# FKGSOFTWARE/TERRA-GAN

Measured on AMD Instinct MI355X. Metric: DSM tiles/sec train-step (G+D) at 256x256 bs=16, higher is better.
Workload: dtype f32; 1 GPU; BASELINE configs[1]: 256x256 1-ch DSM tiles, batch 16 per GPU, fp32, PConv-UNet G + PatchGAN D + L1/VGG-perceptual/TV/boundary(0.5) losses + 2x Adam; global_batch=16, tile=256, parallelism=single-gpu, launch=eager, vgg_weights=deterministic stand-in (ImageNet weights not fetchable offline; same FLOPs), vgg_trunk=forward Winograd F(2x2,3x3), dgrads F(4x4,3x3) (DESIGN 2b)

## Files before the change

### include/terragan_hip.h

```cpp
#ifndef TERRAGAN_HIP_H
#define TERRAGAN_HIP_H

#include <stddef.h>
#include <stdint.h>

#ifdef __cplusplus
extern "C" {
#endif

typedef void* tg_stream_t;

enum { TG_OK = 0, TG_ERR_ARG = -1, TG_ERR_LAUNCH = -2, TG_ERR_WS = -3 };
enum { TG_ACT_NONE = 0, TG_ACT_RELU = 1, TG_ACT_LEAKY = 2 };
enum { TG_PREC_F32 = 0, TG_PREC_BF16 = 1, TG_PREC_F32_WINO4 = 2 };

typedef struct TgConv {
    int32_t B, H, W, Cin;
    int32_t Ho, Wo, Cout;
    int32_t k, stride, pad;
    int32_t precision;
} TgConv;

int tg_version(void);
const char* tg_last_error(void);


size_t tg_conv_fwd_ws_bytes(const TgConv* g);
int tg_conv_fwd(const TgConv* g, const float* x, const float* in_mask, const float* w,
                const float* bias, const float* ratio, int act, float slope, float* y,
                float* ws, size_t ws_bytes, tg_stream_t stream);

size_t tg_conv_dgrad_ws_bytes(const TgConv* g);
int tg_conv_dgrad(const TgConv* g, const float* dy, const float* w, const float* in_mask,
                  float* dx, int accumulate, float* ws, size_t ws_bytes, tg_stream_t stream);
int tg_conv_dgrad_gated(const TgConv* g, const float* dy, const float* w, const float* in_mask,
                        const float* x_act, int act, float slope, float* dx, float* ws,
                        size_t ws_bytes, tg_stream_t stream);

enum { TG_WPREP_FWD = 0, TG_WPREP_DGRAD = 1 };
size_t tg_conv_wprep_bytes(const TgConv* g, int mode);
int tg_conv_wprep(const TgConv* g, int mode, const float* w, float* wprep, tg_stream_t stream);
size_t tg_conv_wprep_item_bytes(void);
int tg_conv_wprep_item(const TgConv* g, int mode, const float* w, float* wprep, void* item_out);
int tg_conv_wprep_run(const void* items_dev, int n, tg_stream_t stream);
int tg_conv_fwd_p(const TgConv* g, const float* x, const float* in_mask, const float* w, const float* wprep,
                  const float* bias, const float* ratio, int act, float slope, float* y, float* ws,
                  size_t ws_bytes, tg_stream_t stream);
int tg_conv_fwd_pool(const TgConv* g, const float* x, const float* in_mask, const float* w, const float* wprep,
                     const float* bias, const float* ratio, int act, float slope, float* y, float* pool_y, float* ws,
                     size_t ws_bytes, tg_stream_t stream);
int tg_conv_pool_code_supported(const TgConv* g);
int tg_conv_fwd_pool_code(const TgConv* g, const float* x, const float* w, const float* wprep, const float* bias,
                          float* pool_y, unsigned char* code, float* ws, size_t ws_bytes, tg_stream_t stream);
int tg_maxpool2_bwd_code(const float* dout, const unsigned char* code, int B, int Ho, int Wo, int C, float* dx,
                         tg_stream_t stream);
typedef struct TgSparseMap {
    const uint32_t* bits;
    const int32_t* list;
    const int32_t* count;
    const uint64_t* pix;
    int32_t nb, tiles_y, tiles_x, _pad;
} TgSparseMap;
size_t tg_vgg_sparse_map_bytes(int nb, int H, int W, const char* plan);
int tg_vgg_sparse_map(const float* x, const float* mask, int nb, int H, int W, const char* plan, void* buf, size_t buf_bytes,
                      int* ticket, TgSparseMap* maps, tg_stream_t stream);
int tg_conv_dgrad_sparse(const TgConv* g, const float* dy, const float* w, const float* wprep, const float* x_act, int act,
                         float slope, const uint32_t* gate_bits, float* dx, const TgSparseMap* sp, float* ws, size_t ws_bytes,
                         tg_stream_t stream);
int tg_conv_dgrad_sparse_planned(const TgConv* g, int gate, const TgSparseMap* sp);
int tg_maxpool2_bwd_code_sparse(const float* dout, const unsigned char* code, int B, int Ho, int Wo, int C, float* dx,
                                const TgSparseMap* sp, tg_stream_t stream);
int tg_conv_fwd_sparse(const TgConv* g, const float* x, const float* w, const float* wprep, const float* bias, int act,
                       float slope, float* y, float* pool_y, unsigned char* code, const TgSparseMap* sp, float* ws,
                       size_t ws_bytes, tg_stream_t stream);
typedef struct TgBnAct {
    const float *mean, *rstd, *gamma, *beta;
    int32_t act;
    float slope;
} TgBnAct;
int tg_conv_bnin_supported(const TgConv* g, int wgrad);
int tg_conv_fwd_bnin(const TgConv* g, const float* x, const TgBnAct* bn, const float* w, const float* bias, int act,
                     float slope, float* y, float* ws, size_t ws_bytes, tg_stream_t stream);
int tg_conv_wgrad_bnin(const TgConv* g, const float* x, const TgBnAct* bn, const float* dy, float* dw, float* db, float* ws,
                       size_t ws_bytes, tg_stream_t stream);
int tg_conv_dgrad_p(const TgConv* g, const float* dy, const float* w, const float* wprep, const float* in_mask,
                    const float* x_act, int act, float slope, float* dx, int accumulate, float* ws,
                    size_t ws_bytes, tg_stream_t stream);
int tg_relu_gate_pack(const float* a, int64_t rows, int C, uint32_t* bits, tg_stream_t stream);
int tg_conv_dgrad_gbits(const TgConv* g, const float* dy, const float* w, const float* wprep, const float* in_mask,
                        const uint32_t* gate_bits, float* dx, int accumulate, float* ws, size_t ws_bytes, tg_stream_t stream);

int tg_set_cu_reserve(int cus);
int tg_set_work_stealing(int mode);

size_t tg_conv_wgrad_ws_bytes(const TgConv* g);
int tg_conv_wgrad(const TgConv* g, const float* x, const float* in_mask, const float* dy,
                  float* dw, float* db, float* ws, size_t ws_bytes, tg_stream_t stream);

int tg_fold_cin(const float* w3, int cout, int taps, int cin, float* w1, tg_stream_t stream);


int tg_mask_update(const float* mask, int B, int H, int W, int k, int stride, int pad, int Ho,
                   int Wo, float* mask_out, float* ratio, tg_stream_t stream);
int tg_mask_up_merge(const float* up_mask, const float* skip_mask, int B, int h, int w, int H,
                     int W, float* out, tg_stream_t stream);

#define TG_MASK_PYRAMID_MAX 24
typedef struct TgMaskOp {
    int kind, H, W, Ho, Wo, k, stride, pad;
    const float* in;
    const float* in2;
    float* out;
    float* out2;
} TgMaskOp;
typedef struct TgMaskPyramid {
    int nops, _pad;
    TgMaskOp op[TG_MASK_PYRAMID_MAX];
} TgMaskPyramid;
int tg_mask_pyramid(const TgMaskPyramid* pm, int B, tg_stream_t stream);


size_t tg_bn_ws_bytes(int64_t rows, int C);
int tg_bn_stats(const float* y, int64_t rows, int C, float eps, float momentum, float* save_mean,
                float* save_rstd, float* running_mean, float* running_var,
                int64_t* num_batches_tracked, float* ws, size_t ws_bytes, tg_stream_t stream);
int tg_bn_fwd(const float* y, int64_t rows, int C, float eps, float momentum, const float* gamma,
              const float* beta, int act, float slope, float* save_mean, float* save_rstd,
              float* running_mean, float* running_var, int64_t* num_batches_tracked, float* out,
              float* ws, size_t ws_bytes, tg_stream_t stream);
int tg_bn_eval_stats(const float* running_mean, const float* running_var, int C, float eps,
                     float* mean, float* rstd, tg_stream_t stream);
int tg_bn_act_fwd(const float* y, int64_t rows, int C, const float* mean, const float* rstd,
                  const float* gamma, const float* beta, int act, float slope, float* out,
                  tg_stream_t stream);
int tg_bn_act_bwd(const float* dout, const float* y, int64_t rows, int C, const float* mean,
                  const float* rstd, const float* gamma, const float* beta, int act, float slope,
                  const float* ratio, float* dy, float* dgamma, float* dbeta, float* dbias, float* ws,
                  size_t ws_bytes, tg_stream_t stream);
int tg_bn_bwd_conv1_supported(int64_t rows, int C);
size_t tg_bn_conv1_ws_bytes(int64_t rows, int C);
int tg_bn_act_bwd_conv1(const float* dz, const float* w, int B, int H, int W, const float* y, int C, const float* mean,
                        const float* rstd, const float* gamma, const float* beta, int act, float slope, const float* ratio,
                        float* dy, float* dgamma, float* dbeta, float* dbias, float* ws, size_t ws_bytes, tg_stream_t stream);
int tg_act_bwd(const float* dout, const float* out, int64_t rows, int C, int act, float slope,
               const float* ratio, float* din, tg_stream_t stream);


int tg_upcat_fwd(const float* up, const float* skip, const float* out_mask, int B, int h, int w,
                 int Cu, int H, int W, int Cs, float* out, tg_stream_t stream);
int tg_upcat_bn_supported(int B, int h, int w, int Cu, int H, int W, int Cs);
int tg_upcat_fwd_bn(const float* up, const TgBnAct* bn, const float* skip, const float* out_mask, int B, int h, int w,
                    int Cu, int H, int W, int Cs, float* out, tg_stream_t stream);
int tg_upcat_bwd(const float* dout, int B, int h, int w, int Cu, int H, int W, int Cs, float* dup,
                 float* dskip, tg_stream_t stream);


int tg_sigmoid_composite_fwd(const float* logits, const float* x, const float* mask, int64_t n,
                             float* out, tg_stream_t stream);
int tg_sigmoid_composite_bwd(const float* dout, const float* logits, const float* mask, int64_t n,
                             float* dlogits, float* dx, tg_stream_t stream);

int tg_maxpool2_fwd(const float* x, int B, int H, int W, int C, float* out, tg_stream_t stream);
int tg_maxpool2_bwd(const float* dout, const float* x, int B, int H, int W, int C, int relu_gate,
                    float* dx, tg_stream_t stream);


size_t tg_pixel_loss_ws_bytes(int B, int H, int W);
int tg_pixel_losses(const float* pred, const float* target, const float* mask,
                    const float* l1_weight, int B, int H, int W,
                    float w_l1, float w_tv, float w_bnd, float bnd_eps, const float* gscale,
                    float* out5, float* dpred, int accumulate, float* ws, size_t ws_bytes,
                    tg_stream_t stream);

size_t tg_reduce_ws_bytes(int64_t n);
int tg_l1_mean(const float* a, const float* b, int64_t n, float coef, const float* gscale,
               float* out1, float* da, float* ws, size_t ws_bytes, tg_stream_t stream);
int tg_l1_mean_relu(const float* a, const float* b, int64_t n, float coef, const float* gscale, float* out1, float* da,
                    float* ws, size_t ws_bytes, tg_stream_t stream);

int tg_bce_logits(const float* z, int64_t n, float target, float coef, const float* gscale,
                  float* out1, float* dz, float* ws, size_t ws_bytes, tg_stream_t stream);


int tg_adam(float* p, const float* g, float* m, float* v, int64_t n, double lr, double beta1,
            double beta2, double eps, int step, float grad_scale, tg_stream_t stream);

typedef struct TgAdamSeg {
    float* p;
    const float* g;
    float* m;
    float* v;
    int64_t n;
} TgAdamSeg;
int tg_adam_multi(const TgAdamSeg* segs_dev, const int32_t* work_dev, int nwork, int chunk_elems,
                  double lr, double beta1, double beta2, double eps, int step, float grad_scale,
                  tg_stream_t stream);

int tg_adam_scalars(double lr, double beta1, double beta2, int step, float* out2_host);
int tg_write_floats(float* dst_dev, int n, const float* vals_host, tg_stream_t stream);
int tg_adam_multi_s(const TgAdamSeg* segs_dev, const int32_t* work_dev, int nwork, int chunk_elems,
                    double beta1, double beta2, double eps, const float* scal_dev, float grad_scale,
                    tg_stream_t stream);

int tg_axpby(const float* x, float a, float b, float* y, int64_t n, tg_stream_t stream);
int tg_lincomb(const float* x, float a, const float* y, float b, float* out, int64_t n,
               tg_stream_t stream);
int tg_mul(const float* a, const float* b, float* out, int64_t n, tg_stream_t stream);
int tg_mul_keep(const float* a, const float* b, float* out, float* a_copy, int64_t n, tg_stream_t stream);
size_t tg_bn_grouped_ws_bytes(int64_t rows_per_group, int groups, int C);
int tg_bn_fwd_grouped(const float* y, int64_t rows_per_group, int groups, int C, float eps, const float* gamma,
                      const float* beta, int act, float slope, float* save_mean, float* save_rstd, float* out,
                      float* ws, size_t ws_bytes, tg_stream_t stream);
int tg_bn_act_bwd_grouped(const float* dout, const float* y, int64_t rows_per_group, int groups, int C,
                          const float* mean, const float* rstd, const float* gamma, const float* beta, int act,
                          float slope, float* dy, float* dgamma, float* dbeta, float* dbias, float* ws,
                          size_t ws_bytes, tg_stream_t stream);
int tg_bn_running_update_multi(const float* save_mean, const float* save_rstd, int64_t rows_per_group, int C,
                               float eps, float momentum, const int* order, int norder, float* running_mean,
                               float* running_var, int64_t* num_batches_tracked, tg_stream_t stream);
int tg_bn_running_update(const float* save_mean, const float* save_rstd, int64_t rows, int C,
                         float eps, float momentum, float* running_mean, float* running_var,
                         int64_t* num_batches_tracked, tg_stream_t stream);
int tg_nchw_to_nhwc(const float* x, int B, int C, int H, int W, float* y, tg_stream_t stream);
int tg_nhwc_to_nchw(const float* x, int B, int C, int H, int W, float* y, tg_stream_t stream);


size_t tg_quality_metrics_ws_bytes(int64_t imgs, int H, int W);
int tg_quality_metrics(const float* pred, const float* target, const float* mask, int64_t imgs, int H, int W,
                       float* out9, float* ws, size_t ws_bytes, tg_stream_t stream);

int tg_u8_to_tiles(const uint8_t* img_u8, const uint8_t* mask_u8, int64_t n, float* img_f32, float* mask_f32,
                   tg_stream_t stream);

typedef struct TgRasterPlan {
    int32_t H, W;
    int32_t wh, ww;
    int32_t overlap;
    int32_t ny, nx;
} TgRasterPlan;

int tg_raster_window_stats(const float* dem, const float* mask, const TgRasterPlan* plan, int use_nodata, float nodata,
                           float* lo, float* hi, int32_t* counts, tg_stream_t stream);
int tg_raster_gather(const float* dem, const float* mask, const TgRasterPlan* plan, int use_nodata, float nodata,
                     const float* lo, const float* hi, const int32_t* win_idx, int n, float* x, float* m, tg_stream_t stream);
int tg_raster_blend(const float* dem, const float* mask, const TgRasterPlan* plan, int use_nodata, float nodata,
                    const float* lo, const float* hi, const int32_t* run_of_window, const float* wout, int n_run, float* out,
                    int32_t* unfilled, tg_stream_t stream);

enum { TG_HOLE_RECT = 0, TG_HOLE_ELLIPSE = 1, TG_HOLE_STROKE = 2 };
int tg_hole_masks(const int32_t* prims, const int32_t* offsets, int n, int side, float* mask, tg_stream_t stream);
// ... 71 lines not shown
```

### terra-gan_amd/csrc/igemm.hip

```cpp
#include <atomic>
#include <stdlib.h>
#include <string.h>

#include <mutex>
#include <vector>

#include "common.h"

struct ProfRec {
    hipEvent_t a, b;
    int kind;
    double flops, bytes;
    int M, N, K, C, splits, cfg;
    char tag[32];
};
static std::mutex g_prof_mu;
static bool g_prof_on = false;
static std::vector<ProfRec> g_prof;
static thread_local char g_prof_tag[32] = "";

struct ProfScope {
    bool on = false;
    ProfRec r{};
    hipStream_t s;
    ProfScope(hipStream_t st, int kind, double flops, double bytes, int M = 0, int N = 0, int K = 0, int C = 0, int splits = 1,
              int cfg = 0)
        : s(st) {
        if (!g_prof_on) return;
        on = true;
        r.kind = kind; r.flops = flops; r.bytes = bytes;
        r.M = M; r.N = N; r.K = K; r.C = C; r.splits = splits; r.cfg = cfg;
        memcpy(r.tag, g_prof_tag, sizeof(r.tag));
        (void)hipEventCreate(&r.a);
        (void)hipEventCreate(&r.b);
        (void)hipEventRecord(r.a, s);
    }
    ~ProfScope() {
        if (!on) return;
        (void)hipEventRecord(r.b, s);
        std::lock_guard<std::mutex> lk(g_prof_mu);
        g_prof.push_back(r);
    }
};

static thread_local double g_alg_scale = 1.0;
struct AlgScale {
    double prev;
    explicit AlgScale(double sc) : prev(g_alg_scale) { g_alg_scale = sc; }
    ~AlgScale() { g_alg_scale = prev; }
};

extern "C" int tg_prof_enable(int on) {
    std::lock_guard<std::mutex> lk(g_prof_mu);
    g_prof_on = on != 0;
    return TG_OK;
}
extern "C" int tg_prof_tag(const char* tag) {
    strncpy(g_prof_tag, tag ? tag : "", sizeof(g_prof_tag) - 1);
    g_prof_tag[sizeof(g_prof_tag) - 1] = 0;
    return TG_OK;
}
extern "C" int tg_prof_dump(const char* path) {
    std::lock_guard<std::mutex> lk(g_prof_mu);
    FILE* f = fopen(path, "w");
    if (!f) { tg_set_error("tg_prof_dump: cannot open %s", path); return TG_ERR_ARG; }
    fprintf(f, "kind,cfg,M,N,K,C,splits,ms,gflop,alg_mb,tag\n");
    for (auto& r : g_prof) {
        (void)hipEventSynchronize(r.b);
        float t = 0.f;
        (void)hipEventElapsedTime(&t, r.a, r.b);
        fprintf(f, "%d,%d,%d,%d,%d,%d,%d,%.5f,%.4f,%.3f,%s\n", r.kind, r.cfg, r.M, r.N, r.K, r.C, r.splits, t, r.flops / 1e9,
                r.bytes / 1e6, r.tag);
    }
    fclose(f);
    return TG_OK;
}
extern "C" int tg_prof_summary(int kind, double* total_ms, int64_t* launches, double* flops, double* bytes) {
    std::lock_guard<std::mutex> lk(g_prof_mu);
    double ms = 0, fl = 0, by = 0;
    int64_t n = 0;
    std::vector<ProfRec> keep;
    for (auto& r : g_prof) {
        if (r.kind != kind) { keep.push_back(r); continue; }
        (void)hipEventSynchronize(r.b);
        float t = 0.f;
        (void)hipEventElapsedTime(&t, r.a, r.b);
        ms += t; fl += r.flops; by += r.bytes; ++n;
        (void)hipEventDestroy(r.a);
        (void)hipEventDestroy(r.b);
    }
    g_prof.swap(keep);
    if (total_ms) *total_ms = ms;
    if (launches) *launches = n;
    if (flops) *flops = fl;
    if (bytes) *bytes = by;
    return TG_OK;
}

#include "igemm_params.h"

struct LdsOptIn {
    std::mutex mu;
    bool done[64] = {};
};
static int lds_opt_in(LdsOptIn& st, const void* kern, size_t lds, const char* who) {
    int dev = 0;
    (void)hipGetDevice(&dev);
    std::lock_guard<std::mutex> lk(st.mu);
    if (dev >= 0 && dev < 64 && st.done[dev]) return TG_OK;
    hipError_t e = hipFuncSetAttribute(kern, hipFuncAttributeMaxDynamicSharedMemorySize, (int)lds);
    if (e != hipSuccess) {
        tg_set_error("%s: hipFuncSetAttribute(%zu) failed: %s", who, lds, hipGetErrorString(e));
        return TG_ERR_LAUNCH;
    }
    if (dev >= 0 && dev < 64) st.done[dev] = true;
    return TG_OK;
}

constexpr int WINO_PLAN_CUS = 256;
static std::atomic<int> g_cu_reserve{0};
static int wino_cus() {
    const int c = 256 - g_cu_reserve.load(std::memory_order_relaxed);
    return c < 8 ? 8 : c;
}
extern "C" int tg_set_cu_reserve(int cus) {
    TG_REQUIRE(cus >= 0 && cus <= 128, "tg_set_cu_reserve: %d out of range [0,128]", cus);
    g_cu_reserve.store(cus, std::memory_order_relaxed);
    return TG_OK;
}

static std::atomic<int> g_work_stealing{0};
extern "C" int tg_set_work_stealing(int mode) {
    TG_REQUIRE(mode >= 0 && mode <= 2, "tg_set_work_stealing: mode %d not in {0, 1, 2}", mode);
    g_work_stealing.store(mode, std::memory_order_relaxed);
    return TG_OK;
}
constexpr int WQ_HOST_Z = 16, WQ_HOST_INTS = 8 * WQ_HOST_Z + 8, WQ_POOL_BLOCKS = 64;
static int* wino_queue_block(hipStream_t s, int splits, int total_work) {
    static const int env_mode = getenv("TG_WORK_STEALING") ? atoi(getenv("TG_WORK_STEALING")) : 0;
    const int set_mode = g_work_stealing.load(std::memory_order_relaxed);
    const int mode = set_mode ? set_mode : env_mode;
    if (mode <= 0 || splits > WQ_HOST_Z) return nullptr;
    if (mode == 1 && total_work < 2 * wino_cus()) return nullptr;
    static std::mutex mu;
    static std::vector<std::pair<std::pair<int, hipStream_t>, int*>> blocks;
    static int* pools[64] = {};
    static int used[64] = {};
    int dev = 0;
    if (hipGetDevice(&dev) != hipSuccess || dev < 0 || dev >= 64) return nullptr;
    std::lock_guard<std::mutex> lk(mu);
    for (auto& b : blocks)
        if (b.first.first == dev && b.first.second == s) return b.second;
    hipStreamCaptureStatus st = hipStreamCaptureStatusNone;
    if (hipStreamIsCapturing(s, &st) != hipSuccess || st != hipStreamCaptureStatusNone) {
        if (!pools[dev]) return nullptr;
    }
    if (!pools[dev]) {
        if (hipMalloc(reinterpret_cast<void**>(&pools[dev]), (size_t)WQ_POOL_BLOCKS * WQ_HOST_INTS * sizeof(int)) != hipSuccess) { pools[dev] = nullptr; return nullptr; }
        if (hipMemset(pools[dev], 0, (size_t)WQ_POOL_BLOCKS * WQ_HOST_INTS * sizeof(int)) != hipSuccess) return nullptr;
    }
    if (used[dev] >= WQ_POOL_BLOCKS) return nullptr;
    int* blk = pools[dev] + (size_t)used[dev]++ * WQ_HOST_INTS;
    blocks.push_back({{dev, s}, blk});
    return blk;
}

static int choose_splits(long tiles, int max_splits, int slots) {
    if (max_splits < 1) max_splits = 1;
    if (tiles >= 4L * slots) return 1;
    int best = 1;
    double best_eff = 0.0;
    for (int sp = 1; sp <= max_splits; ++sp) {
        const long blocks = tiles * sp;
        const long rounds = (blocks + slots - 1) / slots;
        const double eff = (double)blocks / ((double)rounds * slots);
        if (eff > best_eff + 1e-9) { best_eff = eff; best = sp; }
        if (blocks >= slots && eff >= 0.92) return sp;
        if (blocks >= 6L * slots) break;
    }
    return best;
}


static int choose_splits_k(long tiles, int max_splits, int slots, long ksteps, double slab_steps = 0.0) {
    if (max_splits < 1) max_splits = 1;
    int best = 1;
    double best_cost = 1e300;
    for (int sp = 1; sp <= max_splits; ++sp) {
        const long blocks = tiles * sp;
        const long rounds = (blocks + slots - 1) / slots;
        const double cost = (double)rounds * ((double)((ksteps + sp - 1) / sp) + 4.0) + slab_steps * (double)blocks;
        if (cost < best_cost * 0.995) { best_cost = cost; best = sp; }
    }
    return best;
}

__device__ __forceinline__ int cdiv_dev(int a, int b) { return (a + b - 1) / b; }
__device__ __forceinline__ int xcd_remap(int id, int total) {
    const int xcd = id & 7, slot = id >> 3;
    const int qd = total >> 3, rm = total & 7;
    return (xcd < rm ? xcd * (qd + 1) : rm * (qd + 1) + (xcd - rm) * qd) + slot;
}

__device__ __forceinline__ f32x4 epilogue4(const IGemmParams& p, f32x4 o, size_t pix, int nb, const f32x4* gv_pre = nullptr,
                                           const float* rs_pre = nullptr, const f32x4* bias_pre = nullptr) {
    const float rs = rs_pre ? *rs_pre : (p.rowscale ? p.rowscale[pix] : 1.f);
    if (bias_pre) o += *bias_pre;
    else if (p.bias) o += *reinterpret_cast<const f32x4*>(p.bias + nb);
    o *= rs;
#pragma unroll
    for (int e = 0; e < 4; ++e) o[e] = apply_act(o[e], p.act, p.slope);
    if (p.gate) {
        const f32x4 gv = gv_pre ? *gv_pre : *reinterpret_cast<const f32x4*>(p.gate + pix * p.N + nb);
#pragma unroll
        for (int e = 0; e < 4; ++e) o[e] *= gv[e] > 0.f ? 1.f : (p.gate_act == TG_ACT_LEAKY ? p.gate_slope : 0.f);
    }
    if (p.accumulate) o += *reinterpret_cast<const f32x4*>(p.dst + pix * p.N + nb);
    return o;
}

__device__ __forceinline__ size_t dst_pixel(const IGemmParams& p, int m) {
    if (p.ds == 1 && p.OH == p.DH && p.OW == p.DW) return (size_t)m;
    int ox = m % p.OW;
    int t = m / p.OW;
    int oy = t % p.OH;
    int b = t / p.OH;
    return ((size_t)b * p.DH + (oy * p.ds + p.dy0)) * p.DW + (ox * p.ds + p.dx0);
}

template <int WAVES_M, int WAVES_N, int WM, int WN, bool SCALAR, bool BF16>
__device__ __forceinline__ void igemm_body(const IGemmParams& p, const int bz) {
    constexpr int BM = WAVES_M * WM * 32, BN = WAVES_N * WN * 32, LDK = 36;
    constexpr int A_LOADS = BM / 32, B_LOADS = BN / 32;
    static_assert(WAVES_M * WAVES_N == 4, "4 waves per workgroup");
    extern __shared__ __attribute__((aligned(16))) float smem[];
    float* As = smem;
    float* Bs = smem + 2 * BM * LDK;
    constexpr int LDH = 40;
    __bf16* Ah = reinterpret_cast<__bf16*>(smem);
    __bf16* Bh = Ah + 2 * BM * LDH;

    const int tid = threadIdx.x, lane = tid & 63, wave = tid >> 6;
    const int wm = wave / WAVES_N, wn = wave % WAVES_N;
    const int m0 = blockIdx.x * BM, n0 = blockIdx.y * BN;
    if (m0 >= p.M) return;
    const int kc = tid & 7, r0 = tid >> 3;

    int rb[A_LOADS], ry[A_LOADS], rx[A_LOADS];
    bool rv[A_LOADS];
#pragma unroll
    for (int i = 0; i < A_LOADS; ++i) {
        int m = m0 + r0 + 32 * i;
        rv[i] = m < p.M;
        int mm = rv[i] ? m : 0;
        int ox = mm % p.OW;
        int t = mm / p.OW;
        int oy = t % p.OH;
        rb[i] = t / p.OH;
        ry[i] = oy * p.ss + p.sy0;
        rx[i] = ox * p.ss + p.sx0;
    }

    const int t_begin = bz * p.steps_per_split;
    const int t_end = min(p.T, t_begin + p.steps_per_split);

    f32x4 ra[A_LOADS], rw[B_LOADS];
    float rmk[A_LOADS];

    int l_ty = 0, l_tx = 0, l_ch = 0;
    if constexpr (!SCALAR) {
        const int tap0 = t_begin / p.nchunks;
        l_ch = t_begin - tap0 * p.nchunks;
        l_ty = tap0 / p.TW;
        l_tx = tap0 - l_ty * p.TW;
    }
    int g_c0 = 0, g_dyy = 0, g_dxx = 0, g_widx = 0;
    bool g_cv = false;
    auto gbegin = [&]() {
        g_c0 = l_ch * 32 + 4 * kc;
        g_dyy = l_ty * p.tstep;
        g_dxx = l_tx * p.tstep;
        g_widx = ((p.ky0 + l_ty * p.kstep) * p.KW + (p.kx0 + l_tx * p.kstep)) * p.C + g_c0;
        g_cv = g_c0 < p.C;
        if (++l_ch == p.nchunks) {
            l_ch = 0;
            if (++l_tx == p.TW) { l_tx = 0; ++l_ty; }
        }
// ... 924 lines not shown
static size_t align_up(size_t v, size_t a) { return (v + a - 1) / a * a; }
#include "wino22.inc"
static size_t conv_wino_floats(const TgConv* g) {
    if (wino22_fwd_geom_ok(g) || wino22_dgrad_geom_ok(g)) return wino22_u_floats(g);
    if (g->k != 3 || g->stride != 1 || (g->Cin % 8) != 0 || (g->Cout % 8) != 0) return 0;
    if (g->precision == TG_PREC_F32_WINO4) return align_up(wino44_u_floats(g->Cout, g->Cin), 64);
    return align_up(wino_u_floats(g->Cout, g->Cin), 64);
}

__global__ __launch_bounds__(256) void s2d_kernel(const float* __restrict__ x, const float* __restrict__ mask, float* __restrict__ x2,
                                                  int B, int H, int W, int C) {
    const int C4 = C >> 2;
    const int64_t total = (int64_t)B * H * W * C4;
    for (int64_t idx = (int64_t)blockIdx.x * 256 + threadIdx.x; idx < total; idx += (int64_t)gridDim.x * 256) {
        const int c4 = (int)(idx % C4);
        int64_t pix = idx / C4;
        const int xw = (int)(pix % W);
        int64_t t = pix / W;
        const int yh = (int)(t % H);
        const int b = (int)(t / H);
        f32x4 v = *reinterpret_cast<const f32x4*>(x + pix * C + 4 * c4);
        if (mask) v *= mask[pix];
        const int64_t p2 = ((int64_t)b * (H >> 1) + (yh >> 1)) * (W >> 1) + (xw >> 1);
        *reinterpret_cast<f32x4*>(x2 + p2 * (4 * C) + ((yh & 1) * 2 + (xw & 1)) * C + 4 * c4) = v;
    }
}
__global__ __launch_bounds__(256) void d2s_kernel(const float* __restrict__ dx2, const float* __restrict__ mask, float* __restrict__ dx,
                                                  int B, int H, int W, int C, int accumulate) {
    const int C4 = C >> 2;
    const int64_t total = (int64_t)B * H * W * C4;
    for (int64_t idx = (int64_t)blockIdx.x * 256 + threadIdx.x; idx < total; idx += (int64_t)gridDim.x * 256) {
        const int c4 = (int)(idx % C4);
        int64_t pix = idx / C4;
        const int xw = (int)(pix % W);
        int64_t t = pix / W;
        const int yh = (int)(t % H);
        const int b = (int)(t / H);
        const int64_t p2 = ((int64_t)b * (H >> 1) + (yh >> 1)) * (W >> 1) + (xw >> 1);
        f32x4 v = *reinterpret_cast<const f32x4*>(dx2 + p2 * (4 * C) + ((yh & 1) * 2 + (xw & 1)) * C + 4 * c4);
        if (mask) v *= mask[pix];
        float* o = dx + pix * C + 4 * c4;
        if (accumulate) v += *reinterpret_cast<const f32x4*>(o);
        *reinterpret_cast<f32x4*>(o) = v;
    }
}
__global__ __launch_bounds__(256) void w5x5_s2d_kernel(const float* __restrict__ src, float* __restrict__ dst, int Cout, int C, int to3) {
    const int64_t total = to3 ? (int64_t)Cout * 36 * C : (int64_t)Cout * 25 * C;
    for (int64_t idx = (int64_t)blockIdx.x * 256 + threadIdx.x; idx < total; idx += (int64_t)gridDim.x * 256) {
        const int c = (int)(idx % C);
        int64_t t = idx / C;
        if (to3) {
            const int ph = (int)(t % 4), tap = (int)((t / 4) % 9), co = (int)(t / 36);
            const int ky = 2 * (tap / 3) + (ph >> 1), kx = 2 * (tap % 3) + (ph & 1);
            dst[idx] = (ky < 5 && kx < 5) ? src[((int64_t)co * 25 + ky * 5 + kx) * C + c] : 0.f;
        } else {
            const int k = (int)(t % 25), co = (int)(t / 25);
            const int ky = k / 5, kx = k % 5;
            dst[idx] = src[(((int64_t)co * 9 + (ky >> 1) * 3 + (kx >> 1)) * 4 + (ky & 1) * 2 + (kx & 1)) * C + c];
        }
    }
}
static bool s2d_ok(const TgConv* g) {
    static const bool off = getenv("TG_NO_WINO") != nullptr || getenv("TG_NO_S2D") != nullptr;
    if (off || (g->precision == TG_PREC_BF16 && getenv("TG_NO_WINO16"))) return false;
    return g->k == 5 && g->stride == 2 && g->pad == 2 && (g->H % 2) == 0 && (g->W % 2) == 0 && (g->Cin % 16) == 0 &&
           (g->Cout % 64) == 0 && g->Ho >= 32 && g->Wo >= 32 && g->Ho == g->H / 2 && g->Wo == g->W / 2;
}
static TgConv s2d_geom(const TgConv* g) {
    TgConv g2 = *g;
    g2.H = g->H / 2; g2.W = g->W / 2; g2.Cin = 4 * g->Cin; g2.k = 3; g2.stride = 1; g2.pad = 1;
    return g2;
}
static size_t s2d_x_floats(const TgConv* g) { return align_up((size_t)g->B * g->H * g->W * g->Cin, 64); }
static size_t s2d_w_floats(const TgConv* g) { return align_up((size_t)g->Cout * 36 * g->Cin, 64); }

static size_t splitk_room_floats(size_t out) {
    const size_t cap = (size_t)64 << 20;
    return out * 64 < cap ? out * 64 : cap;
}
static size_t min_floats(size_t a, size_t b) { return a < b ? a : b; }

extern "C" size_t tg_conv_fwd_ws_bytes(const TgConv* g) {
    if (!g) return 0;
    const size_t out = (size_t)g->B * g->Ho * g->Wo * g->Cout;
    size_t base = (splitk_room_floats(out) + conv_wino_floats(g)) * sizeof(float);
    if (s2d_ok(g)) {
        const TgConv g2 = s2d_geom(g);
        base = (s2d_x_floats(g) + s2d_w_floats(g)) * sizeof(float) + tg_conv_fwd_ws_bytes(&g2);
    }
    return base;
}

static IGemmParams conv_fwd_params(const TgConv* g) {
    IGemmParams p = {};
    p.B = g->B; p.IH = g->H; p.IW = g->W; p.C = g->Cin;
    p.OH = g->Ho; p.OW = g->Wo; p.N = g->Cout; p.M = g->B * g->Ho * g->Wo;
    p.DH = g->Ho; p.DW = g->Wo; p.ds = 1; p.dy0 = 0; p.dx0 = 0;
    p.TH = g->k; p.TW = g->k; p.ss = g->stride; p.tstep = 1; p.sy0 = -g->pad; p.sx0 = -g->pad;
    p.KW = g->k; p.kstep = 1; p.ky0 = 0; p.kx0 = 0;
    p.Kfull = g->k * g->k * g->Cin;
    p.bf16 = g->precision == TG_PREC_BF16;
    p.wino4 = g->precision == TG_PREC_F32_WINO4;
    p.Ktot = p.TH * p.TW * p.C; p.nchunks = cdiv(p.C, 32);
    p.T = (p.C % 4) ? cdiv(p.Ktot, 32) : p.TH * p.TW * p.nchunks;
    return p;
}
static IGemmParams conv_dgrad_s1_params(const TgConv* g) {
    IGemmParams p = {};
    p.B = g->B; p.IH = g->Ho; p.IW = g->Wo; p.C = g->Cout;
    p.OH = g->H; p.OW = g->W; p.N = g->Cin; p.M = g->B * g->H * g->W;
    p.DH = g->H; p.DW = g->W; p.ds = 1;
    p.ky0 = 0; p.kx0 = 0; p.TH = g->k; p.TW = g->k; p.ss = g->stride; p.tstep = -1; p.sy0 = g->pad; p.sx0 = g->pad;
    p.KW = g->k; p.kstep = 1; p.Kfull = g->k * g->k * g->Cout;
    p.bf16 = g->precision == TG_PREC_BF16;
    p.wino4 = g->precision == TG_PREC_F32_WINO4;
    return p;
}
static bool wino_fwd_geom_ok(const TgConv* g) { return wino_geom_ok(conv_fwd_params(g)); }
static bool wino_dgrad_geom_ok(const TgConv* g) { return wino_geom_ok(conv_dgrad_s1_params(g)); }

static int launch_wino_s1(IGemmParams& p, float* ws, size_t head, size_t avail, size_t room, hipStream_t s, const char* who) {
    if (wino44_ok(p)) {
        TG_REQUIRE(!p.pool_only, "%s: wino44_kernel cannot write the pool in place of the output", who);
        return launch_wino44(p, s);
    }
    if (wino44_prepared_unusable(p)) {
        TG_REQUIRE(ws && aligned16(ws) && avail >= head, "%s: workspace too small to re-prepare the weights (%zu < %zu floats)", who,
                   avail, head);
        p.wino_u = ws;
        p.wino_ready = 0;
        p.ws = ws + head;
        avail -= head;
    }
    return launch_wino(p, min_floats(avail, room), s);
}

static size_t dgrad_wt_floats(const TgConv* g);
extern "C" size_t tg_conv_wprep_bytes(const TgConv* g, int mode) {
    if (!g) return 0;
    if (s2d_ok(g)) {
        const TgConv g2 = s2d_geom(g);
        return s2d_w_floats(g) * sizeof(float) + tg_conv_wprep_bytes(&g2, mode);
    }
    if (mode == TG_WPREP_FWD) return wino_fwd_geom_ok(g) || wino22_fwd_geom_ok(g) ? conv_wino_floats(g) * sizeof(float) : 0;
    if (mode == TG_WPREP_DGRAD) return dgrad_wt_floats(g) * sizeof(float);
    return 0;
}

struct FwdExtras {
    float* pool_dst = nullptr;
    unsigned char* pool_code = nullptr;
    const BnIn* in_bn = nullptr;
    const TgSparseMap* sparse = nullptr;
    int pool_fused = 0;
};
static int conv_fwd_impl(const TgConv* g, const float* x, const float* in_mask, const float* w, float* wprep, int prep,
                         const float* bias, const float* ratio, int act, float slope, float* y, float* ws, size_t ws_bytes,
                         tg_stream_t stream, float* pool_y = nullptr, FwdExtras* ex = nullptr) {
    if (pool_y) {
        TG_REQUIRE(g && x && y && prep >= 0 && (g->Ho % 2) == 0 && (g->Wo % 2) == 0 && aligned16(pool_y),
                   "tg_conv_fwd_pool: even output sizes and a 16-byte aligned pool_y expected");
        int fused = 0;
        if (!s2d_ok(g) && !wino22_fwd_geom_ok(g)) {
            FwdExtras e;
            e.pool_dst = pool_y;
            e.sparse = ex ? ex->sparse : nullptr;
            const int rc1 = conv_fwd_impl(g, x, in_mask, w, wprep, prep, bias, ratio, act, slope, y, ws, ws_bytes, stream, nullptr, &e);
            if (rc1) return rc1;
            fused = e.pool_fused;
        } else if (int rc1 = conv_fwd_impl(g, x, in_mask, w, wprep, prep, bias, ratio, act, slope, y, ws, ws_bytes, stream)) {
            return rc1;
        }
        return fused ? TG_OK : tg_maxpool2_fwd(y, g->B, g->Ho, g->Wo, g->Cout, pool_y, stream);
    }
    int rc = check_conv(g, "tg_conv_fwd");
    if (rc) return rc;
    TG_REQUIRE(w && (prep < 0 || (x && y)), "tg_conv_fwd: null pointer");
    TG_REQUIRE(aligned16(x) && aligned16(w) && aligned16(y) && aligned16(wprep), "tg_conv_fwd: pointers must be 16-byte aligned");
    TG_REQUIRE(prep == 0 || wprep != nullptr, "tg_conv_fwd: prepared weights expected");
    const bool ws_ok = ws && aligned16(ws) && ws_bytes >= tg_conv_fwd_ws_bytes(g);
    if (s2d_ok(g) && (prep < 0 || ws_ok)) {
        hipStream_t s = (hipStream_t)stream;
        const TgConv g2 = s2d_geom(g);
        float* x2 = ws;
        float* w2 = prep ? wprep : ws + s2d_x_floats(g);
        float* ws2 = ws ? ws + s2d_x_floats(g) + s2d_w_floats(g) : nullptr;
        if (prep < 0 && g_wprep_capture) {
            const int rc2 = conv_fwd_impl(&g2, nullptr, nullptr, w2, wprep + s2d_w_floats(g), -1, nullptr, nullptr, 0, 0.f, nullptr, nullptr,
                                          0, stream);
            if (rc2 == TG_OK && g_wprep_captured == 1 && g_wprep_capture->kind == 1) {
                g_wprep_capture->kind = 4; g_wprep_capture->w = w; g_wprep_capture->taps = g->Cin;
            } else {
                g_wprep_captured = -1;
            }
            return rc2;
        }
        if (prep <= 0) {
            hipLaunchKernelGGL(w5x5_s2d_kernel, dim3(ew_grid((int64_t)g->Cout * 36 * g->Cin, 256)), dim3(256), 0, s, w, w2, g->Cout, g->Cin, 1);
            TG_CHECK_LAUNCH("w5x5_s2d_kernel");
        }
        if (prep >= 0) {
            hipLaunchKernelGGL(s2d_kernel, dim3(ew_grid((int64_t)g->B * g->H * g->W * (g->Cin / 4), 256)), dim3(256), 0, s, x, in_mask, x2,
                               g->B, g->H, g->W, g->Cin);
            TG_CHECK_LAUNCH("s2d_kernel");
        }
        AlgScale sc(25.0 / 36.0);
        return conv_fwd_impl(&g2, x2, nullptr, w2, prep ? wprep + s2d_w_floats(g) : nullptr, prep, bias, ratio, act, slope, y, ws2,
                             ws ? ws_bytes - (s2d_x_floats(g) + s2d_w_floats(g)) * sizeof(float) : 0, stream);
    }
    TG_REQUIRE(!(s2d_ok(g) && prep > 0), "tg_conv_fwd: workspace too small for the prepared 5x5 stride-2 path");
    IGemmParams p = conv_fwd_params(g);
    p.src = x; p.amask = in_mask; p.wmat = w; p.bias = bias; p.rowscale = ratio; p.dst = y; p.ws = ws;
    p.act = act; p.slope = slope; p.accumulate = 0;
    size_t ws_floats = ws ? ws_bytes / sizeof(float) : 0;
    const size_t uf = conv_wino_floats(g);
    const size_t room = splitk_room_floats((size_t)p.M * p.N);
    if (wino22_fwd_geom_ok(g) && (prep || (ws_floats >= uf && aligned16(ws)))) {
        p.w_raw = w;
        p.wino_u = prep ? wprep : ws;
        p.wino_ready = prep;
        if (!prep) {
            p.ws = ws + uf;
            ws_floats -= uf;
        }
        return launch_wino22(g, p, 0, min_floats(ws_floats, room), (hipStream_t)stream);
    }
    const bool wino = wino_fwd_geom_ok(g) && (prep || (ws_floats >= uf && aligned16(ws)));
    if (prep < 0 && !wino) return TG_OK;
    if (ex) {
        p.pool_dst = ex->pool_dst;
        p.pool_code = ex->pool_code;
        p.pool_only = ex->pool_code != nullptr;
        p.sparse = ex->sparse;
        if (ex->in_bn) {
            p.in_bn = *ex->in_bn;
            TG_REQUIRE(smallconv_bnin_fwd_ok(p), "tg_conv_fwd_bnin: geometry not supported (ask tg_conv_bnin_supported first)");
        }
    }
    if (wino) {
        p.w_raw = w; p.w_sn = (long)p.Kfull; p.w_sk = 1; p.w_stap = g->Cin;
        p.wino_u = prep ? wprep : ws;
        p.wino_ready = prep;
        if (!prep) {
            p.ws = ws + uf;
            ws_floats -= uf;
        }
        rc = launch_wino_s1(p, ws, uf, ws_floats, room, (hipStream_t)stream, "tg_conv_fwd");
    } else {
        ws_floats = min_floats(ws_floats, room);
        plan_splits(p, ws_floats);
        rc = launch_igemm(p, (hipStream_t)stream, ws_floats);
    }
    if (ex) ex->pool_fused = p.pool_done;
    return rc;
}
extern "C" int tg_conv_fwd_pool(const TgConv* g, const float* x, const float* in_mask, const float* w, const float* wprep,
                                const float* bias, const float* ratio, int act, float slope, float* y, float* pool_y, float* ws,
                                size_t ws_bytes, tg_stream_t stream) {
    TG_REQUIRE(pool_y, "tg_conv_fwd_pool: null pointer");
    return conv_fwd_impl(g, x, in_mask, w, const_cast<float*>(wprep), wprep ? 1 : 0, bias, ratio, act, slope, y, ws, ws_bytes, stream,
                         pool_y);
}
extern "C" int tg_conv_pool_code_supported(const TgConv* g) {
    if (!g || (g->precision != TG_PREC_F32 && g->precision != TG_PREC_BF16) || !wino_fwd_geom_ok(g) || s2d_ok(g) || (g->Ho & 1) ||
        (g->Wo & 1) || getenv("TG_NO_POOL_CODE"))
        return 0;
    IGemmParams p = conv_fwd_params(g);
    float pooled;
    p.pool_dst = &pooled;
    return wino_plan(p, splitk_room_floats((size_t)p.M * p.N)).pool ? 1 : 0;
}
static int conv_fwd_pool_code(const TgConv* g, const float* x, const float* w, const float* wprep, const float* bias, float* pool_y,
                              unsigned char* code, const TgSparseMap* sp, float* ws, size_t ws_bytes, tg_stream_t stream) {
    TG_REQUIRE(pool_y && code && aligned16(pool_y) && (reinterpret_cast<uintptr_t>(code) & 3) == 0, "tg_conv_fwd_pool_code: bad pointers");
    TG_REQUIRE(tg_conv_pool_code_supported(g), "tg_conv_fwd_pool_code: geometry not supported (ask tg_conv_pool_code_supported first)");
    FwdExtras e;
    e.pool_dst = pool_y;
    e.pool_code = code;
    e.sparse = sp;
    const int rc = conv_fwd_impl(g, x, nullptr, w, const_cast<float*>(wprep), wprep ? 1 : 0, bias, nullptr, TG_ACT_RELU, 0.f, pool_y, ws,
                                 ws_bytes, stream, nullptr, &e);
    if (rc) return rc;
    TG_REQUIRE(e.pool_fused, "tg_conv_fwd_pool_code: internal: the launch did not take the fused path");
    return TG_OK;
}
extern "C" int tg_conv_fwd_pool_code(const TgConv* g, const float* x, const float* w, const float* wprep, const float* bias,
                                     float* pool_y, unsigned char* code, float* ws, size_t ws_bytes, tg_stream_t stream) {
    return conv_fwd_pool_code(g, x, w, wprep, bias, pool_y, code, nullptr, ws, ws_bytes, stream);
}
extern "C" int tg_conv_fwd_sparse(const TgConv* g, const float* x, const float* w, const float* wprep, const float* bias, int act,
                                  float slope, float* y, float* pool_y, unsigned char* code, const TgSparseMap* sp, float* ws,
                                  size_t ws_bytes, tg_stream_t stream) {
    if (code) {
        TG_REQUIRE(act == TG_ACT_RELU, "tg_conv_fwd_sparse: the pool code needs a ReLU output");
        return conv_fwd_pool_code(g, x, w, wprep, bias, pool_y, code, sp, ws, ws_bytes, stream);
    }
    FwdExtras e;
    e.sparse = sp;
    return conv_fwd_impl(g, x, nullptr, w, const_cast<float*>(wprep), wprep ? 1 : 0, bias, nullptr, act, slope, y, ws, ws_bytes, stream,
                         pool_y, &e);
}
static bool bnin_geom_ok(const TgConv* g) {
    return g && g->Cout == 1 && g->Cin == 64 && g->k == 3 && g->stride == 1 && g->pad == 1 && (g->Wo % 4) == 0;
}
static BnIn bnin_of(const TgBnAct* bn) { return BnIn{bn->mean, bn->rstd, bn->gamma, bn->beta, bn->act, bn->slope}; }
static WgradParams wgrad_params(const TgConv* g);
extern "C" int tg_conv_bnin_supported(const TgConv* g, int wgrad) {
    if (!bnin_geom_ok(g)) return 0;
    if (wgrad) {
        const WgradParams p = wgrad_params(g);
        return smallconv_wgrad_applies(p) && smallconv_bnin_wgrad_ok(p) ? 1 : 0;
    }
    return smallconv_bnin_fwd_ok(conv_fwd_params(g)) ? 1 : 0;
}
extern "C" int tg_conv_fwd_bnin(const TgConv* g, const float* x, const TgBnAct* bn, const float* w, const float* bias, int act,
                                float slope, float* y, float* ws, size_t ws_bytes, tg_stream_t stream) {
    TG_REQUIRE(bn && bn->mean && bn->rstd && bn->gamma && bn->beta, "tg_conv_fwd_bnin: null pointer");
    TG_REQUIRE(tg_conv_bnin_supported(g, 0), "tg_conv_fwd_bnin: geometry not supported (ask tg_conv_bnin_supported first)");
    const BnIn b = bnin_of(bn);
    FwdExtras e;
    e.in_bn = &b;
    return conv_fwd_impl(g, x, nullptr, w, nullptr, 0, bias, nullptr, act, slope, y, ws, ws_bytes, stream, nullptr, &e);
}
extern "C" int tg_conv_fwd(const TgConv* g, const float* x, const float* in_mask, const float* w, const float* bias,
                           const float* ratio, int act, float slope, float* y, float* ws, size_t ws_bytes,
                           tg_stream_t stream) {
    return conv_fwd_impl(g, x, in_mask, w, nullptr, 0, bias, ratio, act, slope, y, ws, ws_bytes, stream);
}
extern "C" int tg_conv_fwd_p(const TgConv* g, const float* x, const float* in_mask, const float* w, const float* wprep,
                             const float* bias, const float* ratio, int act, float slope, float* y, float* ws, size_t ws_bytes,
                             tg_stream_t stream) {
    return conv_fwd_impl(g, x, in_mask, w, const_cast<float*>(wprep), wprep ? 1 : 0, bias, ratio, act, slope, y, ws, ws_bytes,
                         stream);
}

__global__ __launch_bounds__(256) void transpose_w_kernel(const float* __restrict__ w, float* __restrict__ wt,
                                                          int cout, int taps, int cin) {
    const size_t total = (size_t)cout * taps * cin;
    for (size_t idx = (size_t)blockIdx.x * 256 + threadIdx.x; idx < total; idx += (size_t)gridDim.x * 256) {
        int co = (int)(idx % cout);
        size_t r = idx / cout;
        int t = (int)(r % taps);
        int ci = (int)(r / taps);
        wt[idx] = w[((size_t)co * taps + t) * cin + ci];
    }
}

static size_t dgrad_wt_floats(const TgConv* g) {
    size_t wt = align_up((size_t)g->Cout * g->k * g->k * g->Cin, 64);
    size_t uf = conv_wino_floats(g);
    return wt > uf ? wt : uf;
}
extern "C" size_t tg_conv_dgrad_ws_bytes(const TgConv* g) {
    if (!g) return 0;
    if (s2d_ok(g)) {
        const TgConv g2 = s2d_geom(g);
        return (s2d_x_floats(g) + s2d_w_floats(g)) * sizeof(float) + tg_conv_dgrad_ws_bytes(&g2);
    }
    return (dgrad_wt_floats(g) + splitk_room_floats((size_t)g->B * g->H * g->W * g->Cin)) * sizeof(float);
}

static int conv_dgrad_impl(const TgConv* g, const float* dy, const float* w, float* wprep, int prep, const float* in_mask, float* dx,
                           int accumulate, const float* gate, int gate_act, float gate_slope, float* ws, size_t ws_bytes,
                           tg_stream_t stream, const uint32_t* gate_bits = nullptr, int* gate_bits_done = nullptr,
                           const TgSparseMap* sparse = nullptr, int* sparse_pix_done = nullptr);
extern "C" int tg_conv_dgrad(const TgConv* g, const float* dy, const float* w, const float* in_mask, float* dx,
                             int accumulate, float* ws, size_t ws_bytes, tg_stream_t stream) {
    return conv_dgrad_impl(g, dy, w, nullptr, 0, in_mask, dx, accumulate, nullptr, 0, 0.f, ws, ws_bytes, stream);
}
extern "C" int tg_conv_dgrad_gated(const TgConv* g, const float* dy, const float* w, const float* in_mask, const float* x_act,
                                   int act, float slope, float* dx, float* ws, size_t ws_bytes, tg_stream_t stream) {
    TG_REQUIRE(x_act != nullptr && (act == TG_ACT_RELU || act == TG_ACT_LEAKY), "tg_conv_dgrad_gated: needs x_act and a ReLU/LeakyReLU");
    return conv_dgrad_impl(g, dy, w, nullptr, 0, in_mask, dx, 0, x_act, act, slope, ws, ws_bytes, stream);
}
extern "C" int tg_conv_dgrad_p(const TgConv* g, const float* dy, const float* w, const float* wprep, const float* in_mask,
                               const float* x_act, int act, float slope, float* dx, int accumulate, float* ws, size_t ws_bytes,
                               tg_stream_t stream) {
    TG_REQUIRE(x_act == nullptr || ((act == TG_ACT_RELU || act == TG_ACT_LEAKY) && !accumulate),
               "tg_conv_dgrad_p: a gated dgrad needs a ReLU/LeakyReLU and accumulate == 0");
    const bool usable = wprep != nullptr && !(x_act != nullptr && g && s2d_ok(g));
    return conv_dgrad_impl(g, dy, w, usable ? const_cast<float*>(wprep) : nullptr, usable ? 1 : 0, in_mask, dx, accumulate, x_act,
                           act, slope, ws, ws_bytes, stream);
}
extern "C" int tg_conv_dgrad_gbits(const TgConv* g, const float* dy, const float* w, const float* wprep, const float* in_mask,
                                   const uint32_t* gate_bits, float* dx, int accumulate, float* ws, size_t ws_bytes, tg_stream_t stream) {
    int rc = check_conv(g, "tg_conv_dgrad_gbits");
    if (rc) return rc;
    TG_REQUIRE(dy && w && gate_bits && dx && ws, "tg_conv_dgrad_gbits: null pointer");
    TG_REQUIRE(!accumulate, "tg_conv_dgrad_gbits: a gated dgrad does not accumulate");
    TG_REQUIRE(g->Cin % 32 == 0, "tg_conv_dgrad_gbits: needs Cin %% 32 == 0 (one gate word per 32 channels), got %d", g->Cin);
    TG_REQUIRE((reinterpret_cast<uintptr_t>(gate_bits) & 15) == 0, "tg_conv_dgrad_gbits: pointers must be 16-byte aligned");
    const bool usable = wprep != nullptr && !s2d_ok(g);
    int done = 0;
    rc = conv_dgrad_impl(g, dy, w, usable ? const_cast<float*>(wprep) : nullptr, usable ? 1 : 0, in_mask, dx, 0, nullptr, TG_ACT_NONE, 0.f,
                         ws, ws_bytes, stream, gate_bits, &done);
    if (rc || done) return rc;
    return gate_bits_apply_launch(dx, gate_bits, (int64_t)g->B * g->H * g->W, g->Cin, (hipStream_t)stream);
}
extern "C" int tg_conv_dgrad_sparse(const TgConv* g, const float* dy, const float* w, const float* wprep, const float* x_act, int act,
                                    float slope, const uint32_t* gate_bits, float* dx, const TgSparseMap* sp, float* ws, size_t ws_bytes,
                                    tg_stream_t stream) {
    int rc = check_conv(g, "tg_conv_dgrad_sparse");
    if (rc) return rc;
    TG_REQUIRE(dy && w && dx && ws && sp, "tg_conv_dgrad_sparse: null pointer");
    TG_REQUIRE(sp->nb == g->B, "tg_conv_dgrad_sparse: the map describes %d images, the batch has %d", sp->nb, g->B);
    TG_REQUIRE(!(x_act && gate_bits), "tg_conv_dgrad_sparse: x_act and gate_bits are exclusive");
    TG_REQUIRE(x_act == nullptr || act == TG_ACT_RELU || act == TG_ACT_LEAKY, "tg_conv_dgrad_sparse: a gated dgrad needs a ReLU/LeakyReLU");
    TG_REQUIRE(g->Cin != 1 || sp->pix, "tg_conv_dgrad_sparse: Cin == 1 needs a map built with a mask (sp->pix)");
    if (gate_bits) {
        TG_REQUIRE(g->Cin % 32 == 0, "tg_conv_dgrad_sparse: gate_bits need Cin %% 32 == 0, got %d", g->Cin);
        TG_REQUIRE((reinterpret_cast<uintptr_t>(gate_bits) & 15) == 0, "tg_conv_dgrad_sparse: pointers must be 16-byte aligned");
    }
    const bool usable = wprep != nullptr && !s2d_ok(g);
    int bits_done = 0, pix_done = 0;
    rc = conv_dgrad_impl(g, dy, w, usable ? const_cast<float*>(wprep) : nullptr, usable ? 1 : 0, nullptr, dx, 0, x_act,
                         x_act ? act : TG_ACT_NONE, slope, ws, ws_bytes, stream, gate_bits, &bits_done, sp, &pix_done);
    if (rc) return rc;
    if (gate_bits && !bits_done) rc = gate_bits_apply_launch(dx, gate_bits, (int64_t)g->B * g->H * g->W, g->Cin, (hipStream_t)stream);
    if (rc) return rc;
    if (g->Cin == 1 && !pix_done) return pix_zero_launch(dx, sp->pix, g->B, g->H, g->W, (hipStream_t)stream);
    return TG_OK;
}
extern "C" int tg_conv_dgrad_sparse_planned(const TgConv* g, int gate, const TgSparseMap* sp) {
    if (!g || !sp || gate < 0 || gate > 2 || check_conv(g, "tg_conv_dgrad_sparse_planned") || !wino_dgrad_geom_ok(g)) return 0;
    static const float some_gate = 0.f;
    static const uint32_t some_bits = 0;
    IGemmParams p = conv_dgrad_s1_params(g);
    p.act = TG_ACT_NONE;
    p.gate = gate == 1 ? &some_gate : nullptr; p.gate_act = TG_ACT_RELU;
    p.gate_bits = gate == 2 ? &some_bits : nullptr;
    p.sparse = sp;
    if (wino44_ok(p)) return 0;
    return wino_plan(p, splitk_room_floats((size_t)g->B * g->H * g->W * g->Cin)).sparse_list ? 1 : 0;
}
extern "C" int tg_conv_wprep(const TgConv* g, int mode, const float* w, float* wprep, tg_stream_t stream) {
    TG_REQUIRE(g && w && wprep, "tg_conv_wprep: null pointer");
    TG_REQUIRE(mode == TG_WPREP_FWD || mode == TG_WPREP_DGRAD, "tg_conv_wprep: bad mode %d", mode);
    TG_REQUIRE(tg_conv_wprep_bytes(g, mode) > 0, "tg_conv_wprep: this (geometry, mode) runs on the raw weights");
    if (mode == TG_WPREP_FWD)
        return conv_fwd_impl(g, nullptr, nullptr, w, wprep, -1, nullptr, nullptr, 0, 0.f, nullptr, nullptr, 0, stream);
    return conv_dgrad_impl(g, nullptr, w, wprep, -1, nullptr, nullptr, 0, nullptr, 0, 0.f, nullptr, 0, stream);
}
extern "C" size_t tg_conv_wprep_item_bytes(void) { return sizeof(TgWprepItem); }
extern "C" int tg_conv_wprep_item(const TgConv* g, int mode, const float* w, float* wprep, void* item_out) {
    if (!g || !w || !wprep || !item_out || (mode != TG_WPREP_FWD && mode != TG_WPREP_DGRAD)) return 0;
    if (tg_conv_wprep_bytes(g, mode) == 0) return 0;
    TgWprepItem it = {};
    g_wprep_capture = &it;
    g_wprep_captured = 0;
    int rc = mode == TG_WPREP_FWD ? conv_fwd_impl(g, nullptr, nullptr, w, wprep, -1, nullptr, nullptr, 0, 0.f, nullptr, nullptr, 0, nullptr)
                                  : conv_dgrad_impl(g, nullptr, w, wprep, -1, nullptr, nullptr, 0, nullptr, 0, 0.f, nullptr, 0, nullptr);
    g_wprep_capture = nullptr;
    if (rc != TG_OK || g_wprep_captured != 1) return 0;
    memcpy(item_out, &it, sizeof(it));
    return 1;
}
extern "C" int tg_conv_wprep_run(const void* items_dev, int n, tg_stream_t stream) {
    TG_REQUIRE(items_dev && n > 0, "tg_conv_wprep_run: bad arguments");
    hipLaunchKernelGGL(wprep_multi_kernel, dim3(2048, n), dim3(256), 0, (hipStream_t)stream, static_cast<const TgWprepItem*>(items_dev));
    TG_CHECK_LAUNCH("wprep_multi_kernel");
    return TG_OK;
}
static int conv_dgrad_impl(const TgConv* g, const float* dy, const float* w, float* wprep, int prep, const float* in_mask, float* dx,
                           int accumulate, const float* gate, int gate_act, float gate_slope, float* ws, size_t ws_bytes,
                           tg_stream_t stream, const uint32_t* gate_bits, int* gate_bits_done, const TgSparseMap* sparse,
                           int* sparse_pix_done) {
    int rc = check_conv(g, "tg_conv_dgrad");
    if (rc) return rc;
    TG_REQUIRE(w && (prep < 0 || (dy && dx && ws)), "tg_conv_dgrad: null pointer");
    TG_REQUIRE(aligned16(dy) && aligned16(w) && aligned16(dx) && aligned16(ws) && aligned16(wprep),
               "tg_conv_dgrad: pointers must be 16-byte aligned");
    TG_REQUIRE(prep == 0 || wprep != nullptr, "tg_conv_dgrad: prepared weights expected");
    if (s2d_ok(g) && gate == nullptr && gate_bits == nullptr && (prep < 0 || ws_bytes >= tg_conv_dgrad_ws_bytes(g))) {
        hipStream_t s2 = (hipStream_t)stream;
        const TgConv g2 = s2d_geom(g);
        float* dx2 = ws;
        float* w2 = prep ? wprep : ws + s2d_x_floats(g);
        float* wsr = ws ? ws + s2d_x_floats(g) + s2d_w_floats(g) : nullptr;
        if (prep < 0 && g_wprep_capture) {
            const int rc2 = conv_dgrad_impl(&g2, nullptr, w2, wprep + s2d_w_floats(g), -1, nullptr, nullptr, 0, nullptr, 0, 0.f, nullptr, 0, stream);
            if (rc2 == TG_OK && g_wprep_captured == 1 && g_wprep_capture->kind == 1) {
                g_wprep_capture->kind = 4; g_wprep_capture->w = w; g_wprep_capture->taps = g->Cin;
            } else {
                g_wprep_captured = -1;
            }
            return rc2;
// ... 501 lines not shown
                for (int i = 0; i < WM; ++i)
#pragma unroll
                    for (int j = 0; j < WN; ++j) acc[i][j] = __builtin_amdgcn_mfma_f32_32x32x16_bf16(ah[i], bh[j], acc[i][j], 0, 0, 0);
            }
            if (more) sstore(cur ^ 1);
            __syncthreads();
        }
    }
    float* out = p.out + (size_t)bz * p.Cout * p.Ktot;
    if ((p.Ktot & 3) == 0) {
        float* scratch = smem + wave * (32 * 36);
#pragma unroll
        for (int i = 0; i < WM; ++i)
#pragma unroll
            for (int j = 0; j < WN; ++j)
                tile_rows4(scratch, acc[i][j], lane, [&](int rr, int cc, f32x4 v4) {
                    const int co = c0m + (wm * WM + i) * 32 + rr;
                    const int n = n0 + (wn * WN + j) * 32 + cc;
                    if (co < p.Cout && n < p.Ktot) *reinterpret_cast<f32x4*>(out + (size_t)co * p.Ktot + n) = v4;
                });
        return;
    }
#pragma unroll
    for (int i = 0; i < WM; ++i)
#pragma unroll
        for (int r = 0; r < 16; ++r) {
            const int row = (r & 3) + 8 * (r >> 2) + 4 * (lane >> 5);
            const int co = c0m + (wm * WM + i) * 32 + row;
            if (co >= p.Cout) continue;
#pragma unroll
            for (int j = 0; j < WN; ++j) {
                const int n = n0 + (wn * WN + j) * 32 + (lane & 31);
                if (n < p.Ktot) out[(size_t)co * p.Ktot + n] = acc[i][j][r];
            }
        }
}

template <int WAVES_M, int WAVES_N, int WM, int WN>
static int launch_wgrad_bf16_cfg(const WgradParams& p, hipStream_t s) {
    constexpr int BM = WAVES_M * WM * 32, BN = WAVES_N * WN * 32;
    constexpr size_t lds = (size_t)2 * (BM + BN) * 40 * 2;
    WgradParams pp = p;
    pp.rowseg = 1;
    pp.nx = cdiv(p.Ktot, BN);
    pp.ny = cdiv(p.Cout, BM);
    dim3 grid(pp.nx * pp.ny * p.splits);
    {
        const double by = 4.0 * ((double)p.B * p.H * p.W * p.C + (double)p.Mpix * p.Cout + (double)p.Cout * p.Ktot +
                                 (double)p.Mpix + (p.amask ? (double)p.B * p.H * p.W : 0.0));
        ProfScope ps(s, 3, 2.0 * p.Mpix * (double)p.Cout * p.Ktot, by, p.Cout, p.Ktot, p.Mpix, p.C, p.splits, 3500 + BM);
        hipLaunchKernelGGL((wgrad_bf16_kernel<WAVES_M, WAVES_N, WM, WN>), grid, dim3(256), lds, s, pp);
    }
    TG_CHECK_LAUNCH("wgrad_bf16_kernel");
    return TG_OK;
}

__global__ __launch_bounds__(256) void slab_reduce_kernel(const float* __restrict__ ws, float* __restrict__ out,
                                                          size_t n, int splits) {
    if ((n & 3) == 0) {
        const size_t n4 = n >> 2;
        for (size_t idx = (size_t)blockIdx.x * 256 + threadIdx.x; idx < n4; idx += (size_t)gridDim.x * 256) {
            f32x4 v = {0.f, 0.f, 0.f, 0.f};
#pragma unroll 8
            for (int z = 0; z < splits; ++z) v += reinterpret_cast<const f32x4*>(ws + (size_t)z * n)[idx];
            reinterpret_cast<f32x4*>(out)[idx] = v;
        }
        return;
    }
    for (size_t idx = (size_t)blockIdx.x * 256 + threadIdx.x; idx < n; idx += (size_t)gridDim.x * 256) {
        float v = 0.f;
        for (int z = 0; z < splits; ++z) v += ws[(size_t)z * n + idx];
        out[idx] = v;
    }
}

template <int WAVES_M, int WAVES_N, int WM, int WN, bool SA, bool SB>
static int launch_wgrad_cfg(const WgradParams& p, hipStream_t s) {
    constexpr int BM = WAVES_M * WM * 32, BN = WAVES_N * WN * 32;
    constexpr size_t lds = (size_t)2 * 32 * (BM + BN) * sizeof(float);
    static LdsOptIn opt;
    auto kern = wgrad_kernel<WAVES_M, WAVES_N, WM, WN, SA, SB>;
    if (int rc = lds_opt_in(opt, reinterpret_cast<const void*>(kern), lds, "wgrad")) return rc;
    WgradParams pp = p;
    pp.rowseg = (p.Wo % 32 == 0 && !SB && !getenv("TG_NO_ROWSEG")) ? 1 : 0;
    pp.nx = cdiv(p.Ktot, BN);
    pp.ny = cdiv(p.Cout, BM);
    dim3 grid(pp.nx * pp.ny * p.splits);
    {
        const double by = 4.0 * ((double)p.B * p.H * p.W * p.C + (double)p.Mpix * p.Cout + (double)p.Cout * p.Ktot +
                                 (double)p.Mpix + (p.amask ? (double)p.B * p.H * p.W : 0.0));
        ProfScope ps(s, 1, 2.0 * p.Mpix * (double)p.Cout * p.Ktot, by, p.Cout, p.Ktot, p.Mpix, p.C, p.splits, BM);
        hipLaunchKernelGGL(kern, grid, dim3(256), lds, s, pp);
    }
    TG_CHECK_LAUNCH("wgrad_kernel");
    return TG_OK;
}

static int wgrad_bm(const TgConv* g) {
    if (g->Cout % 4 != 0 || g->Cout < 32) return 32;
    if (g->Cout >= 128 && g->Cin % 4 == 0) return 128;
    return 64;
}
static void wgrad_plan(const TgConv* g, int* splits, int* steps_per_split, int* T) {
    const int Mpix = g->B * g->Ho * g->Wo;
    const int Ktot = g->k * g->k * g->Cin;
    const int bm = wgrad_bm(g);
    const long tiles = (long)cdiv(g->Cout, bm) * cdiv(Ktot, 128);
    *T = cdiv(Mpix, 32);
    int smax = cdiv(*T, 4) < 512 ? cdiv(*T, 4) : 512;
    int sp = choose_splits(tiles, smax, 256 * (bm == 128 ? 2 : 3));
    *steps_per_split = cdiv(*T, sp);
    *splits = cdiv(*T, *steps_per_split);
}

int tg_colsum_launch(const float* x, int64_t rows, int C, float* out, float* ws, hipStream_t s);
size_t tg_colsum_ws_floats(int64_t rows, int C);

static WgradParams wgrad_params(const TgConv* g) {
    WgradParams p = {};
    p.B = g->B; p.H = g->H; p.W = g->W; p.C = g->Cin; p.Ho = g->Ho; p.Wo = g->Wo; p.Cout = g->Cout;
    p.k = g->k; p.stride = g->stride; p.pad = g->pad;
    p.Mpix = g->B * g->Ho * g->Wo; p.Ktot = g->k * g->k * g->Cin;
    wgrad_plan(g, &p.splits, &p.steps_per_split, &p.T);
    return p;
}

extern "C" size_t tg_conv_wgrad_ws_bytes(const TgConv* g) {
    if (!g) return 0;
    const WgradParams sp = wgrad_params(g);
    size_t slabs = align_up((size_t)sp.splits * g->Cout * g->k * g->k * g->Cin, 64);
    {
        size_t wf = align_up(wino_wgrad_ws_floats(g), 64);
        if (wf > slabs) slabs = wf;
        wf = align_up(wino22_wgrad_ws_floats(g), 64);
        if (wf > slabs) slabs = wf;
        wf = align_up(wino16_wgrad_ws_floats(g), 64);
        if (wf > slabs) slabs = wf;
    }
    if (s2d_ok(g)) {
        const TgConv g2 = s2d_geom(g);
        size_t wf = s2d_x_floats(g) + s2d_w_floats(g) + align_up(wino_wgrad_ws_floats(&g2), 64);
        if (wino_wgrad_ok(&g2, nullptr) && wf > slabs) slabs = wf;
        wf = s2d_x_floats(g) + s2d_w_floats(g) + align_up(wino16_wgrad_ws_floats(&g2), 64);
        if (wino16_wgrad_ok(&g2, nullptr) && wf > slabs) slabs = wf;
    }
    if (smallconv_wgrad_applies(sp)) {
        size_t alt = align_up(smallconv_wgrad_ws_floats(sp), 64);
        if (alt > slabs) slabs = alt;
    }
    return (slabs + tg_colsum_ws_floats((int64_t)g->B * g->Ho * g->Wo, g->Cout)) * sizeof(float);
}

static int conv_wgrad_impl(const TgConv* g, const float* x, const float* in_mask, const float* dy, float* dw, float* db, float* ws,
                           size_t ws_bytes, tg_stream_t stream, const BnIn* in_bn);
extern "C" int tg_conv_wgrad(const TgConv* g, const float* x, const float* in_mask, const float* dy, float* dw,
                             float* db, float* ws, size_t ws_bytes, tg_stream_t stream) {
    return conv_wgrad_impl(g, x, in_mask, dy, dw, db, ws, ws_bytes, stream, nullptr);
}
extern "C" int tg_conv_wgrad_bnin(const TgConv* g, const float* x, const TgBnAct* bn, const float* dy, float* dw, float* db, float* ws,
                                  size_t ws_bytes, tg_stream_t stream) {
    TG_REQUIRE(bn && bn->mean && bn->rstd && bn->gamma && bn->beta, "tg_conv_wgrad_bnin: null pointer");
    TG_REQUIRE(tg_conv_bnin_supported(g, 1), "tg_conv_wgrad_bnin: geometry not supported (ask tg_conv_bnin_supported first)");
    const BnIn b = bnin_of(bn);
    return conv_wgrad_impl(g, x, nullptr, dy, dw, db, ws, ws_bytes, stream, &b);
}
static int conv_wgrad_impl(const TgConv* g, const float* x, const float* in_mask, const float* dy, float* dw, float* db, float* ws,
                           size_t ws_bytes, tg_stream_t stream, const BnIn* in_bn) {
    int rc = check_conv(g, "tg_conv_wgrad");
    if (rc) return rc;
    TG_REQUIRE(x && dy && dw && ws, "tg_conv_wgrad: null pointer");
    TG_REQUIRE(aligned16(x) && aligned16(dy) && aligned16(dw) && aligned16(ws), "tg_conv_wgrad: pointers must be 16-byte aligned");
    TG_REQUIRE(ws_bytes >= tg_conv_wgrad_ws_bytes(g), "tg_conv_wgrad: workspace too small (%zu < %zu)", ws_bytes,
               tg_conv_wgrad_ws_bytes(g));
    hipStream_t s = (hipStream_t)stream;
    const size_t ws_floats = ws_bytes / sizeof(float);
    const int64_t mpix = (int64_t)g->B * g->Ho * g->Wo;
    auto colsum = [&](size_t off) -> int {
        TG_REQUIRE(off + tg_colsum_ws_floats(mpix, g->Cout) <= ws_floats,
                   "tg_conv_wgrad: workspace too small for the bias column sum (%zu < %zu floats)", ws_floats,
                   off + tg_colsum_ws_floats(mpix, g->Cout));
        return tg_colsum_launch(dy, mpix, g->Cout, db, ws + off, s);
    };
    WgradParams p = wgrad_params(g);
    p.x = x; p.amask = in_mask; p.dy = dy;
    if (in_bn) {
        p.in_bn = *in_bn;
        TG_REQUIRE(smallconv_wgrad_applies(p) && smallconv_bnin_wgrad_ok(p), "tg_conv_wgrad_bnin: geometry not supported");
    }
    if (smallconv_wgrad_applies(p)) {
        int db_done = 0;
        {
            const double by = 4.0 * ((double)p.B * p.H * p.W * p.C + (double)p.Mpix * p.Cout + (double)p.Cout * p.Ktot);
            ProfScope ps(s, 2, 2.0 * p.Mpix * (double)p.Cout * p.Ktot, by, p.Cout, p.Ktot, p.Mpix, p.C, 1, 2001);
            rc = smallconv_wgrad_launch(p, dw, ws, ws_floats, s, db, &db_done);
        }
        if (rc) return rc;
        if (db && !db_done) {
            rc = colsum(align_up(smallconv_wgrad_ws_floats(p), 64));
            if (rc) return rc;
        }
        return TG_OK;
    }
    if (s2d_ok(g)) {
        const TgConv g2 = s2d_geom(g);
        const bool w16 = wino16_wgrad_ok(&g2, nullptr);
        if (w16 || wino_wgrad_ok(&g2, nullptr)) {
            float* x2 = ws;
            float* dw2 = ws + s2d_x_floats(g);
            float* wsr = dw2 + s2d_w_floats(g);
            hipLaunchKernelGGL(s2d_kernel, dim3(ew_grid((int64_t)g->B * g->H * g->W * (g->Cin / 4), 256)), dim3(256), 0, s, x, in_mask,
                               x2, g->B, g->H, g->W, g->Cin);
            TG_CHECK_LAUNCH("s2d_kernel");
            WgradParams p2 = p;
            p2.x = x2; p2.amask = nullptr; p2.H = g2.H; p2.W = g2.W; p2.C = g2.Cin; p2.k = 3; p2.stride = 1; p2.pad = 1;
            p2.Ktot = 9 * g2.Cin;
            {
                AlgScale sc(25.0 / 36.0);
                rc = w16 ? launch_wino16_wgrad(&g2, p2, dw2, wsr, s) : launch_wino_wgrad(&g2, p2, dw2, wsr, s);
            }
            if (rc) return rc;
            hipLaunchKernelGGL(w5x5_s2d_kernel, dim3(ew_grid((int64_t)g->Cout * 25 * g->Cin, 256)), dim3(256), 0, s, dw2, dw, g->Cout,
                               g->Cin, 0);
            TG_CHECK_LAUNCH("w5x5_s2d_kernel");
            if (db) {
                rc = colsum((size_t)(wsr - ws) + align_up(w16 ? wino16_wgrad_ws_floats(&g2) : wino_wgrad_ws_floats(&g2), 64));
                if (rc) return rc;
            }
            return TG_OK;
        }
    }
    if (wino16_wgrad_ok(g, in_mask)) {
        rc = launch_wino16_wgrad(g, p, dw, ws, s);
        if (rc) return rc;
        if (db) {
            rc = colsum(align_up(wino16_wgrad_ws_floats(g), 64));
            if (rc) return rc;
        }
        return TG_OK;
    }
    if (wino_wgrad_ok(g, in_mask)) {
        rc = launch_wino_wgrad(g, p, dw, ws, s);
        if (rc) return rc;
        if (db) {
            rc = colsum(align_up(wino_wgrad_ws_floats(g), 64));
            if (rc) return rc;
        }
        return TG_OK;
    }
    if (wino22_wgrad_ok(g, in_mask)) {
        rc = launch_wino22_wgrad(g, p, dw, ws, s);
        if (rc) return rc;
        if (db) {
            rc = colsum(align_up(wino22_wgrad_ws_floats(g), 64));
            if (rc) return rc;
        }
        return TG_OK;
    }
    p.out = p.splits > 1 ? ws : dw;
    const int bm = wgrad_bm(g);
    const bool sb = (g->Cin % 4) != 0;
    const bool bf = g->precision == TG_PREC_BF16 && !sb && g->Cout % 4 == 0 && g->Wo % 32 == 0 && bm >= 64 && !getenv("TG_NO_BF16_WGRAD");
    if (bf && bm == 128) rc = launch_wgrad_bf16_cfg<2, 2, 2, 2>(p, s);
    else if (bf) rc = launch_wgrad_bf16_cfg<1, 4, 2, 1>(p, s);
    else if (bm == 128) rc = launch_wgrad_cfg<2, 2, 2, 2, false, false>(p, s);
    else if (bm == 64) rc = sb ? launch_wgrad_cfg<1, 4, 2, 1, false, true>(p, s) : launch_wgrad_cfg<1, 4, 2, 1, false, false>(p, s);
    else rc = sb ? launch_wgrad_cfg<1, 4, 1, 1, true, true>(p, s) : launch_wgrad_cfg<1, 4, 1, 1, true, false>(p, s);
    if (rc) return rc;
    const size_t n = (size_t)g->Cout * p.Ktot;
    if (p.splits > 1) {
        hipLaunchKernelGGL(slab_reduce_kernel, dim3(ew_grid((int64_t)((n & 3) ? n : n / 4), 256)), dim3(256), 0, s, ws, dw, n, p.splits);
        TG_CHECK_LAUNCH("slab_reduce_kernel");
    }
    if (db) {
        rc = colsum(align_up((size_t)p.splits * n, 64));
        if (rc) return rc;
    }
    return TG_OK;
}

__global__ __launch_bounds__(256) void fold_cin_kernel(const float* __restrict__ w3, float* __restrict__ w1, int n, int cin) {
    for (int idx = blockIdx.x * 256 + threadIdx.x; idx < n; idx += gridDim.x * 256) {
        float v = 0.f;
        for (int c = 0; c < cin; ++c) v += w3[(size_t)idx * cin + c];
        w1[idx] = v;
    }
}
extern "C" int tg_fold_cin(const float* w3, int cout, int taps, int cin, float* w1, tg_stream_t stream) {
    TG_REQUIRE(w3 && w1 && cout > 0 && taps > 0 && cin > 0, "tg_fold_cin: bad arguments");
    int n = cout * taps;
    hipLaunchKernelGGL(fold_cin_kernel, dim3(ew_grid(n, 256)), dim3(256), 0, (hipStream_t)stream, w3, w1, n, cin);
    TG_CHECK_LAUNCH("fold_cin_kernel");
    return TG_OK;
}
```

### terra-gan_amd/csrc/wino.inc

```
#pragma once
#include <utility>

struct WinoGeom {
    int tiles_x, tiles_y, total_work, chunks_per_split, nt;
    int sy_min, sx_min;
    int interleave;
    int* qctr;
    const uint32_t* sp_bits;
    const int* sp_list;
    const int* sp_count;
    int sp_tiles, sp_nb;
};
struct WinoWeights {
    long sn, sk, stap;
    int kyu[3], kxv[3];
    int k_fast;
};
typedef unsigned int u32x4 __attribute__((ext_vector_type(4)));
constexpr int WINO_BN = 64;
constexpr int WINO_V = 16 * 64 * 8;
constexpr int WINO_U = 16 * WINO_BN * 8;
constexpr int WINO_PPIX = 18 * 18;
constexpr int WINO_P = WINO_PPIX * 8;
constexpr int WINO_LDS_FLOATS = 2 * WINO_V + 2 * WINO_U + WINO_P;
// ... 972 lines not shown
    };
    auto raw_store = [&]() {
#pragma unroll
        for (int i = 0; i < 3; ++i)
            if (xs_on[i]) *reinterpret_cast<f32x4*>(Xr + xs_lds[i]) = rx[i];
        *reinterpret_cast<f32x4*>(Dr + ds_lds) = rd;
    };
    f32x4 xr[2][4], dr[2][2], tt[4], rr[2];
    auto x_read = [&](int j) {
        xr[0][j] = *reinterpret_cast<const f32x4*>(Xr + xrd0 + j * WG_PITCH);
        xr[1][j] = *reinterpret_cast<const f32x4*>(Xr + xrd1 + j * WG_PITCH);
    };
    auto d_read = [&](int i) {
        dr[i][0] = *reinterpret_cast<const f32x4*>(Dr + drd + (i * 16) * WG_PITCH);
        dr[i][1] = *reinterpret_cast<const f32x4*>(Dr + drd + (i * 16 + 1) * WG_PITCH);
    };
    auto x_rows = [&]() {
#pragma unroll
        for (int j = 0; j < 4; ++j) tt[j] = xr[0][j] + xr[1][j] * xs1;
    };
    auto d_rows = [&]() {
#pragma unroll
        for (int j = 0; j < 2; ++j) rr[j] = dr[0][j] * dc0 + dr[1][j] * dc1;
    };
    auto x_out = [&](int buf, int b, int h) {
        const f32x4 v = b == 0 ? tt[0] - tt[2] : b == 1 ? tt[1] + tt[2] : b == 2 ? tt[2] - tt[1] : tt[1] - tt[3];
        float* dst = Bs + buf * WINO_V + b * 512;
        dst[icol[2 * h]] = v[2 * h];
        dst[icol[2 * h + 1]] = v[2 * h + 1];
    };
    auto d_out = [&](int buf, int b, int h) {
        const f32x4 v = b == 0 ? rr[0] : b == 1 ? rr[0] + rr[1] : b == 2 ? rr[0] - rr[1] : -rr[1];
        float* dst = As + buf * WINO_V + b * 512;
        dst[icol[2 * h]] = v[2 * h];
        dst[icol[2 * h + 1]] = v[2 * h + 1];
    };

    const int arow = 32 * mw + (lane & 31), brow = 32 * nw + (lane & 31);
    const int a_off = (8 * xh) * 512 + arow * 8 + ((((lane >> 5) ^ (arow >> 4)) & 1) << 2);
    const int b_off = (8 * xh) * 512 + brow * 8 + ((((lane >> 5) ^ (brow >> 4)) & 1) << 2);

    f32x16 acc[8];
#pragma unroll
    for (int i = 0; i < 8; ++i)
#pragma unroll
        for (int r = 0; r < 16; ++r) acc[i][r] = 0.f;

    if (s_begin < s_end) {
        raw_load();
        raw_store();
        raw_load();
        wino_barrier();
#pragma unroll
        for (int j = 0; j < 4; ++j) x_read(j);
        d_read(0);
        d_read(1);
        x_rows();
        d_rows();
#pragma unroll
        for (int b = 0; b < 4; ++b) { x_out(0, b, 0); x_out(0, b, 1); d_out(0, b, 0); d_out(0, b, 1); }
        wino_barrier();
        f32x4 fa[2], fb[2];
        fa[0] = *reinterpret_cast<const f32x4*>(As + a_off);
        fb[0] = *reinterpret_cast<const f32x4*>(Bs + b_off);
        int cur = 0;
        for (int s = s_begin; s < s_end; ++s) {
            const int nxt = cur ^ 1;
            const float* Ac = As + cur * WINO_V + a_off;
            const float* Bc = Bs + cur * WINO_V + b_off;
            const float* An = As + nxt * WINO_V + a_off;
            const float* Bn = Bs + nxt * WINO_V + b_off;
            wino_static_for(std::make_integer_sequence<int, 32>{}, [&](auto tc) {
                constexpr int t = decltype(tc)::value;
                constexpr int xi = t >> 2, e = t & 3;
                if constexpr (t == 0) raw_store();
                if constexpr (t == 1) raw_load();
                if constexpr (t == 3) wino_barrier();
                if constexpr (t >= 4 && t < 8) x_read(t - 4);
                if constexpr (t == 8) { d_read(0); d_read(1); }
                if constexpr (t == 9) x_rows();
                if constexpr (t >= 10 && t < 18) x_out(nxt, (t - 10) >> 1, t & 1);
                if constexpr (t == 17) d_rows();
                if constexpr (t >= 18 && t < 26) d_out(nxt, (t - 18) >> 1, t & 1);
                if constexpr (t == 27) wino_barrier();
                if constexpr (e == 0 && xi < 7) {
                    fa[(xi + 1) & 1] = *reinterpret_cast<const f32x4*>(Ac + (xi + 1) * 512);
                    fb[(xi + 1) & 1] = *reinterpret_cast<const f32x4*>(Bc + (xi + 1) * 512);
                }
                if constexpr (e == 0 && xi == 7) {
                    fa[0] = *reinterpret_cast<const f32x4*>(An);
                    fb[0] = *reinterpret_cast<const f32x4*>(Bn);
                }
                __builtin_amdgcn_sched_barrier(0);
                acc[xi] = __builtin_amdgcn_mfma_f32_32x32x2f32(fa[xi & 1][e], fb[xi & 1][e], acc[xi], 0, 0, 0);
                __builtin_amdgcn_sched_barrier(0);
            });
            cur = nxt;
        }
    }
    float* slab = slabs + ((size_t)work * 16 + 8 * xh) * 4096;
#pragma unroll
    for (int i = 0; i < 8; ++i)
#pragma unroll
        for (int r = 0; r < 16; ++r) {
            const int row = 32 * mw + (r & 3) + 8 * (r >> 2) + 4 * (lane >> 5);
            slab[(size_t)i * 4096 + row * 64 + 32 * nw + (lane & 31)] = acc[i][r];
        }
}

__global__ __launch_bounds__(256) void wino_wgrad_reduce_kernel(const float* __restrict__ slabs, float* __restrict__ dw, int Cout,
                                                                int Cin, int ntco, int ntci, int splits) {
    const int total = Cout * Cin;
    for (int idx = blockIdx.x * 256 + threadIdx.x; idx < total; idx += gridDim.x * 256) {
        const int col = idx & 63, row = (idx >> 6) & 63, tile = idx >> 12;
        const int tco = tile % ntco, tci = tile / ntco;
        float u[16];
#pragma unroll
        for (int i = 0; i < 16; ++i) u[i] = 0.f;
        const size_t sstride = (size_t)ntci * ntco * 16 * 4096;
        const float* sl = slabs + ((size_t)tile * 16) * 4096 + row * 64 + col;
        int sp = 0;
        for (; sp + 4 <= splits; sp += 4) {
            float v[4][16];
#pragma unroll
            for (int k = 0; k < 4; ++k)
#pragma unroll
                for (int i = 0; i < 16; ++i) v[k][i] = sl[(size_t)(sp + k) * sstride + (size_t)i * 4096];
#pragma unroll
            for (int k = 0; k < 4; ++k)
#pragma unroll
                for (int i = 0; i < 16; ++i) u[i] += v[k][i];
        }
        for (; sp < splits; ++sp)
#pragma unroll
            for (int i = 0; i < 16; ++i) u[i] += sl[(size_t)sp * sstride + (size_t)i * 4096];
        float t[3][4];
#pragma unroll
        for (int b = 0; b < 4; ++b) {
            t[0][b] = u[0 * 4 + b] + 0.5f * (u[1 * 4 + b] + u[2 * 4 + b]);
            t[1][b] = 0.5f * (u[1 * 4 + b] - u[2 * 4 + b]);
            t[2][b] = 0.5f * (u[1 * 4 + b] + u[2 * 4 + b]) + u[3 * 4 + b];
        }
        const int co = tco * 64 + 4 * (row & 15) + (row >> 4), ci = tci * 64 + 4 * (col & 15) + (col >> 4);
        float* o = dw + ((size_t)co * 9) * Cin + ci;
#pragma unroll
        for (int uu = 0; uu < 3; ++uu) {
            o[(size_t)(uu * 3 + 0) * Cin] = t[uu][0] + 0.5f * (t[uu][1] + t[uu][2]);
            o[(size_t)(uu * 3 + 1) * Cin] = 0.5f * (t[uu][1] - t[uu][2]);
            o[(size_t)(uu * 3 + 2) * Cin] = 0.5f * (t[uu][1] + t[uu][2]) + t[uu][3];
        }
    }
}

static bool wino_wgrad_ok(const TgConv* g, const float* in_mask) {
    static const bool off = getenv("TG_NO_WINO") != nullptr || getenv("TG_NO_WINO_WGRAD") != nullptr;
    if (off || in_mask != nullptr) return false;
    if (g->precision == TG_PREC_BF16 && g->Cin > 256) return false;
    if (g->k != 3 || g->stride != 1 || (g->Cin % 64) != 0 || (g->Cout % 64) != 0 || g->Ho < 16 || g->Wo < 16) return false;
    if ((size_t)g->B * g->H * g->W * g->Cin * 4 >= ((size_t)1 << 31) || (size_t)g->B * g->Ho * g->Wo * g->Cout * 4 >= ((size_t)1 << 31))
        return false;
    return true;
}
static WinoWgradGeom wino_wgrad_plan(const TgConv* g) {
    WinoWgradGeom q = {};
    q.strips_x = cdiv(g->Wo, 16);
    q.tiles_y = cdiv(g->Ho, 2);
    q.nstrips = g->B * q.tiles_y * q.strips_x;
    q.ntco = g->Cout / 64;
    q.ntci = g->Cin / 64;
    const int tiles = q.ntco * q.ntci;
    int smax = q.nstrips / 8 < 512 ? q.nstrips / 8 : 512;
    if (smax < 1) smax = 1;
    const int splits = choose_splits_k(tiles, smax, WINO_PLAN_CUS, q.nstrips, 0.03);
    q.steps_per_split = cdiv(q.nstrips, splits);
    q.splits = cdiv(q.nstrips, q.steps_per_split);
    return q;
}
static size_t wino_wgrad_ws_floats(const TgConv* g) {
    if (!wino_wgrad_ok(g, nullptr)) return 0;
    const WinoWgradGeom q = wino_wgrad_plan(g);
    return (size_t)q.splits * q.ntco * q.ntci * 16 * 4096;
}
static int launch_wino_wgrad(const TgConv* g, const WgradParams& p, float* dw, float* ws, hipStream_t s) {
    const WinoWgradGeom q = wino_wgrad_plan(g);
    const size_t lds = (size_t)WINO_WG_LDS_FLOATS * sizeof(float);
    static LdsOptIn opt;
    if (int rc = lds_opt_in(opt, reinterpret_cast<const void*>(wino_wgrad_kernel), lds, "wino wgrad")) return rc;
    {
        const double by = 4.0 * ((double)p.B * p.H * p.W * p.C + (double)p.Mpix * p.Cout + (double)p.Cout * p.Ktot);
        ProfScope ps(s, 1, 2.0 * p.Mpix * (double)p.Cout * p.Ktot * g_alg_scale, by, p.Cout, p.Ktot, p.Mpix, p.C, q.splits, 4164);
        hipLaunchKernelGGL(wino_wgrad_kernel, dim3(q.ntco * q.ntci * q.splits), dim3(WINO_THREADS), lds, s, p, q, ws);
    }
    TG_CHECK_LAUNCH("wino_wgrad_kernel");
    hipLaunchKernelGGL(wino_wgrad_reduce_kernel, dim3(ew_grid((int64_t)g->Cout * g->Cin, 256)), dim3(256), 0, s, ws, dw, g->Cout,
                       g->Cin, q.ntco, q.ntci, q.splits);
    TG_CHECK_LAUNCH("wino_wgrad_reduce_kernel");
    return TG_OK;
}
```

### terra-gan_amd/csrc/wino16.inc

```
#pragma once

constexpr int W16_IMG = 16 * 64 * 16;
constexpr int W16_P = WINO_PPIX * 16;
constexpr size_t W16_LDS_BYTES = 4 * (size_t)W16_IMG * 2 + (size_t)W16_P * 4;
constexpr int W16_PP = WINO_PPIX * 24;
constexpr size_t W16_PIPE_LDS_BYTES = 4 * (size_t)W16_IMG * 2 + (size_t)W16_PP * 4;

__host__ __device__ __forceinline__ int w16_pos(int row, int c) { return ((((c >> 3) ^ (row >> 4)) & 1) << 3) + (c & 7); }

__device__ void wino_weights16_body(const float* __restrict__ w, __bf16* __restrict__ U, int N, int K, const WinoWeights& ww) {
    const int NT = N / WINO_BN, K2 = K >> 1;
    const size_t total = (size_t)N * K2;
    for (size_t idx = (size_t)blockIdx.x * 256 + threadIdx.x; idx < total; idx += (size_t)gridDim.x * 256) {
        int n, k2;
        if (ww.k_fast) { k2 = (int)(idx % K2); n = (int)(idx / K2); }
        else { n = (int)(idx % N); k2 = (int)(idx / N); }
        float u[2][16];
#pragma unroll
        for (int h = 0; h < 2; ++h) {
            const float* wp = w + (size_t)n * ww.sn + (size_t)(2 * k2 + h) * ww.sk;
            float g[3][3];
#pragma unroll
            for (int a = 0; a < 3; ++a)
#pragma unroll
// ... 598 lines not shown
        xs_on[i] = ps < 4 * 34;
        xs_r[i] = ps / 34;
        xs_px[i] = ps - xs_r[i] * 34;
        xs_lds[i] = ps * WG_PITCH + 4 * (((idx & 15) + (xs_px[i] >> 2)) & 15);
    }
    const uint32_t xs_ch = (uint32_t)(tci * 64 + 4 * (tid & 15)) * 4u;
    int ds_i[2], ds_px[2], ds_lds[2];
#pragma unroll
    for (int i = 0; i < 2; ++i) {
        const int idx = tid + WINO_THREADS * i;
        const int ps = idx >> 4;
        ds_i[i] = ps >> 5;
        ds_px[i] = ps & 31;
        ds_lds[i] = ps * WG_PITCH + 4 * (((idx & 15) + (ds_px[i] >> 2)) & 15);
    }
    const uint32_t ds_ch = (uint32_t)(tco * 64 + 4 * (tid & 15)) * 4u;

    f32x4 rx[5], rd[2];
    int ls = s_begin, lsx = s_begin % q.strips_x, lty = (s_begin / q.strips_x) % q.tiles_y, lb = s_begin / (q.strips_x * q.tiles_y);
    auto raw_load = [&]() {
        const bool live = ls < s_end;
#pragma unroll
        for (int i = 0; i < 5; ++i) {
            const int py = 2 * lty - p.pad + xs_r[i], px = 32 * lsx - p.pad + xs_px[i];
            const bool ok = live && xs_on[i] && py >= 0 && py < p.H && px >= 0 && px < p.W;
            const uint32_t off = ok ? (((uint32_t)(lb * p.H + py) * p.W + px) * (uint32_t)p.C) * 4u + xs_ch : OOB;
            rx[i] = __builtin_bit_cast(f32x4, __builtin_amdgcn_raw_buffer_load_b128(xrsrc, off, 0, 0));
        }
#pragma unroll
        for (int i = 0; i < 2; ++i) {
            const int oy = 2 * lty + ds_i[i], ox = 32 * lsx + ds_px[i];
            const bool ok = live && oy < p.Ho && ox < p.Wo;
            const uint32_t off = ok ? (((uint32_t)(lb * p.Ho + oy) * p.Wo + ox) * (uint32_t)p.Cout) * 4u + ds_ch : OOB;
            rd[i] = __builtin_bit_cast(f32x4, __builtin_amdgcn_raw_buffer_load_b128(drsrc, off, 0, 0));
        }
        ++ls;
        if (++lsx == q.strips_x) { lsx = 0; if (++lty == q.tiles_y) { lty = 0; ++lb; } }
    };
    auto raw_store = [&]() {
#pragma unroll
        for (int i = 0; i < 5; ++i)
            if (xs_on[i]) *reinterpret_cast<f32x4*>(Xr + xs_lds[i]) = rx[i];
#pragma unroll
        for (int i = 0; i < 2; ++i) *reinterpret_cast<f32x4*>(Dr + ds_lds[i]) = rd[i];
    };
    typedef __bf16 bf16x2 __attribute__((ext_vector_type(2)));
    auto put = [&](__bf16* img, int b, const f32x4& v0, const f32x4& v1) {
#pragma unroll
        for (int e = 0; e < 4; ++e) {
            bf16x2 w;
            w[0] = (__bf16)v0[e];
            w[1] = (__bf16)v1[e];
            *reinterpret_cast<bf16x2*>(img + b * 1024 + icol[e]) = w;
        }
    };
    auto transform = [&]() {
        {
            f32x4 tt[6];
#pragma unroll
            for (int j = 0; j < 6; ++j) {
                const int px = 4 * kp + j;
                const f32x4 d0 = *reinterpret_cast<const f32x4*>(Xr + (r0 * 34 + px) * WG_PITCH + rq(px));
                const f32x4 d1 = *reinterpret_cast<const f32x4*>(Xr + (r1 * 34 + px) * WG_PITCH + rq(px));
                tt[j] = d0 + d1 * xs1;
            }
            put(Bh, 0, tt[0] - tt[2], tt[2] - tt[4]);
            put(Bh, 1, tt[1] + tt[2], tt[3] + tt[4]);
            put(Bh, 2, tt[2] - tt[1], tt[4] - tt[3]);
            put(Bh, 3, tt[1] - tt[3], tt[3] - tt[5]);
        }
        {
            f32x4 rr[4];
#pragma unroll
            for (int j = 0; j < 4; ++j) {
                const int px = 4 * kp + j;
                const f32x4 d0 = *reinterpret_cast<const f32x4*>(Dr + px * WG_PITCH + rq(px));
                const f32x4 d1 = *reinterpret_cast<const f32x4*>(Dr + (32 + px) * WG_PITCH + rq(px));
                rr[j] = a == 0 ? d0 : a == 1 ? d0 + d1 : a == 2 ? d0 - d1 : -d1;
            }
            put(Ah, 0, rr[0], rr[2]);
            put(Ah, 1, rr[0] + rr[1], rr[2] + rr[3]);
            put(Ah, 2, rr[0] - rr[1], rr[2] - rr[3]);
            put(Ah, 3, -rr[1], -rr[3]);
        }
    };

    const int arow = 32 * mw + (lane & 31), brow = 32 * nw + (lane & 31);
    const int a_off = (8 * xh) * 1024 + arow * 16 + ((((lane >> 5) ^ (arow >> 4)) & 1) << 3);
    const int b_off = (8 * xh) * 1024 + brow * 16 + ((((lane >> 5) ^ (brow >> 4)) & 1) << 3);

    f32x16 acc[8];
#pragma unroll
    for (int i = 0; i < 8; ++i)
#pragma unroll
        for (int r = 0; r < 16; ++r) acc[i][r] = 0.f;

    if (s_begin < s_end) {
        raw_load();
        raw_store();
        raw_load();
        for (int s = s_begin; s < s_end; ++s) {
            wino_barrier();
            transform();
            wino_barrier();
            raw_store();
            raw_load();
#pragma unroll
            for (int xi = 0; xi < 8; ++xi) {
                const bf16x8 fa = *reinterpret_cast<const bf16x8*>(Ah + a_off + xi * 1024);
                const bf16x8 fb = *reinterpret_cast<const bf16x8*>(Bh + b_off + xi * 1024);
                acc[xi] = __builtin_amdgcn_mfma_f32_32x32x16_bf16(fa, fb, acc[xi], 0, 0, 0);
            }
        }
    }
    float* slab = slabs + ((size_t)work * 16 + 8 * xh) * 4096;
#pragma unroll
    for (int i = 0; i < 8; ++i)
#pragma unroll
        for (int r = 0; r < 16; ++r) {
            const int row = 32 * mw + (r & 3) + 8 * (r >> 2) + 4 * (lane >> 5);
            slab[(size_t)i * 4096 + row * 64 + 32 * nw + (lane & 31)] = acc[i][r];
        }
}

static bool wino16_wgrad_ok(const TgConv* g, const float* in_mask) {
    static const bool off = getenv("TG_NO_WINO") != nullptr || getenv("TG_NO_WINO_WGRAD") != nullptr || getenv("TG_NO_WINO16") != nullptr ||
                            getenv("TG_NO_WINO16_WGRAD") != nullptr;
    if (off || in_mask != nullptr || g->precision != TG_PREC_BF16) return false;
    if (g->k != 3 || g->stride != 1 || (g->Cin % 64) != 0 || (g->Cout % 64) != 0 || g->Ho < 16 || g->Wo < 32) return false;
    if ((size_t)g->B * g->H * g->W * g->Cin * 4 >= ((size_t)1 << 31) || (size_t)g->B * g->Ho * g->Wo * g->Cout * 4 >= ((size_t)1 << 31))
        return false;
    return true;
}
static WinoWgradGeom wino16_wgrad_plan(const TgConv* g) {
    WinoWgradGeom q = {};
    q.strips_x = cdiv(g->Wo, 32);
    q.tiles_y = cdiv(g->Ho, 2);
    q.nstrips = g->B * q.tiles_y * q.strips_x;
    q.ntco = g->Cout / 64;
    q.ntci = g->Cin / 64;
    const int tiles = q.ntco * q.ntci;
    int smax = q.nstrips / 4 < 512 ? q.nstrips / 4 : 512;
    if (smax < 1) smax = 1;
    const int splits = choose_splits_k(tiles, smax, WINO_PLAN_CUS, q.nstrips, 0.03);
    q.steps_per_split = cdiv(q.nstrips, splits);
    q.splits = cdiv(q.nstrips, q.steps_per_split);
    return q;
}
static size_t wino16_wgrad_ws_floats(const TgConv* g) {
    if (!wino16_wgrad_ok(g, nullptr)) return 0;
    const WinoWgradGeom q = wino16_wgrad_plan(g);
    return (size_t)q.splits * q.ntco * q.ntci * 16 * 4096;
}
static int launch_wino16_wgrad(const TgConv* g, const WgradParams& p, float* dw, float* ws, hipStream_t s) {
    const WinoWgradGeom q = wino16_wgrad_plan(g);
    static LdsOptIn opt;
    if (int rc = lds_opt_in(opt, reinterpret_cast<const void*>(wino16_wgrad_kernel), W16G_LDS_BYTES, "wino16 wgrad")) return rc;
    {
        const double by = 4.0 * ((double)p.B * p.H * p.W * p.C + (double)p.Mpix * p.Cout + (double)p.Cout * p.Ktot);
        ProfScope ps(s, 3, 2.0 * p.Mpix * (double)p.Cout * p.Ktot * g_alg_scale, by, p.Cout, p.Ktot, p.Mpix, p.C, q.splits, 4116);
        hipLaunchKernelGGL(wino16_wgrad_kernel, dim3(q.ntco * q.ntci * q.splits), dim3(WINO_THREADS), W16G_LDS_BYTES, s, p, q, ws);
    }
    TG_CHECK_LAUNCH("wino16_wgrad_kernel");
    hipLaunchKernelGGL(wino_wgrad_reduce_kernel, dim3(ew_grid((int64_t)g->Cout * g->Cin, 256)), dim3(256), 0, s, ws, dw, g->Cout,
                       g->Cin, q.ntco, q.ntci, q.splits);
    TG_CHECK_LAUNCH("wino_wgrad_reduce_kernel");
    return TG_OK;
}
```

### terra-gan_amd/tg_hip/engine.py

```python
import os
from types import SimpleNamespace as NS

import torch

from . import ops as O

G_ENC = [("enc1", 1, 64, 7, 2, 3), ("enc2", 64, 128, 5, 2, 2), ("enc3", 128, 256, 5, 2, 2),
         ("enc4", 256, 512, 3, 2, 1), ("enc5", 512, 512, 3, 2, 1), ("enc6", 512, 512, 3, 2, 1),
         ("enc7", 512, 512, 3, 2, 1)]
G_DEC = [("dec7", 1024, 512, 3, 1, 1), ("dec6", 1024, 512, 3, 1, 1), ("dec5", 1024, 512, 3, 1, 1),
         ("dec4", 768, 256, 3, 1, 1), ("dec3", 384, 128, 3, 1, 1), ("dec2", 192, 64, 3, 1, 1),
         ("dec1", 64, 64, 3, 1, 1)]
D_LAYERS = [(0, None, None, 64, 4, 2, 1, True), (2, 3, 64, 128, 4, 2, 1, True), (5, 6, 128, 256, 4, 2, 1, True),
            (8, 9, 256, 512, 4, 2, 1, True), (11, None, 512, 1, 4, 1, 1, False)]
VGG_TRUNK = [0, 2, "M", 5, 7, "M", 10, 12, 14]


VGG_WINO4 = os.environ.get("TG_VGG_WINO4", "1") != "0"
VGG_WINO4_FWD = os.environ.get("TG_VGG_WINO4_FWD", "0") == "1"
VGG_WINO4_MINCH = int(os.environ.get("TG_VGG_WINO4_MINCH", "128"))
VGG_SPARSE = os.environ.get("TG_VGG_SPARSE", "1") != "0"
VGG_SPARSE_BWD = os.environ.get("TG_VGG_SPARSE_BWD", "1") != "0"
POOL_CODE = os.environ.get("TG_NO_POOL_CODE") is None


def _vgg_wino4(w, B, H, W, cout, mode=None, default=True):
    if mode is False or (mode is None and not default):
        return False
    wide = max(w.shape[0], w.shape[1]) >= VGG_WINO4_MINCH
    if mode is True:
        return wide
    items = B * ((H + 15) // 16) * ((W + 31) // 32) * (cout // 64)
    return wide and items >= 256
_side = {}
SIDE_WGRAD = os.environ.get("TG_SIDE_STREAM") == "1"
PROBE = None


def _side_stream():
    dev = torch.cuda.current_device()
    st = _side.get(dev)
    if st is None:
        st = _side[dev] = torch.cuda.Stream(device=dev)
    return st


def _wgrad(gbuf, inputs, fn):
    if gbuf is None or not SIDE_WGRAD:
        return fn()
    main, side = torch.cuda.current_stream(), _side_stream()
    side.wait_stream(main)
    with torch.cuda.stream(side):
        out = fn()
    for t in inputs:
        if t is not None:
            t.record_stream(side)
    return out


def join_side():
    if SIDE_WGRAD and torch.cuda.current_device() in _side:
        torch.cuda.current_stream().wait_stream(_side_stream())


def _pconv_fwd(P, name, k, s, p, x, in_mask, ratio, training, premasked=False, defer_act=False):
    O.tag(f"{name}.fwd")
    y = O.conv_fwd(x, P[f"{name}.input_conv.weight"], P[f"{name}.input_conv.bias"].detach(), k, s, p,
                   in_mask=None if premasked else in_mask, ratio=ratio)
    if training:
        mean, rstd, a = O.bn_fwd(y, P[f"{name}.bn.weight"], P[f"{name}.bn.bias"], O.ACT_RELU, 0.0, P[f"{name}.bn.running_mean"],
                                 P[f"{name}.bn.running_var"], P[f"{name}.bn.num_batches_tracked"], apply=not defer_act)
    else:
        mean, rstd = O.bn_eval_stats(P[f"{name}.bn.running_mean"], P[f"{name}.bn.running_var"])
        a = None if defer_act else O.bn_act_fwd(y, mean, rstd, P[f"{name}.bn.weight"], P[f"{name}.bn.bias"], O.ACT_RELU)
    if PROBE is not None:
        PROBE("fwd", name, a if a is not None else O.bn_act_fwd(y, mean, rstd, P[f"{name}.bn.weight"], P[f"{name}.bn.bias"], O.ACT_RELU))
    return a, NS(name=name, k=k, s=s, p=p, x=x, in_mask=in_mask, ratio=ratio, y=y, mean=mean, rstd=rstd,
                 premasked=premasked)


def _notify(on_ready, grads, keys):
    if on_ready is not None and not SIDE_WGRAD:
        for k in keys:
            on_ready(k, grads[k])


def _pconv_bwd(P, c, da, grads, dx_out=None, want_dx=True, gbuf=None, on_ready=None, conv1=None):
    name = c.name
    if PROBE is not None:
        PROBE("bwd", name, da)
    outs = (gbuf[f"{name}.bn.weight"], gbuf[f"{name}.bn.bias"], gbuf[f"{name}.input_conv.bias"]) if gbuf is not None else None
    if conv1 is not None:
        dyr, dgamma, dbeta, db = O.bn_act_bwd_conv1(conv1[0], conv1[1], c.y, c.mean, c.rstd, P[f"{name}.bn.weight"], P[f"{name}.bn.bias"],
                                                    O.ACT_RELU, ratio=c.ratio, outs=outs)
    else:
        dyr, dgamma, dbeta, db = O.bn_act_bwd(da, c.y, c.mean, c.rstd, P[f"{name}.bn.weight"], P[f"{name}.bn.bias"], O.ACT_RELU,
                                              ratio=c.ratio, outs=outs)
    O.tag(f"{name}.dgrad")
    dx = O.conv_dgrad(dyr, P[f"{name}.input_conv.weight"], tuple(c.x.shape), c.k, c.s, c.p, in_mask=c.in_mask, out=dx_out) \
        if want_dx else None
    wmask = None if getattr(c, "premasked", False) else c.in_mask
    O.tag(f"{name}.wgrad")
    dw, _ = _wgrad(gbuf, (c.x, dyr, wmask), lambda: O.conv_wgrad(
        c.x, dyr, P[f"{name}.input_conv.weight"], c.k, c.s, c.p, in_mask=wmask, want_bias=False,
        dw_out=gbuf[f"{name}.input_conv.weight"] if gbuf is not None else None))
    grads[f"{name}.input_conv.weight"], grads[f"{name}.input_conv.bias"] = dw, db
    grads[f"{name}.bn.weight"], grads[f"{name}.bn.bias"] = dgamma, dbeta
    _notify(on_ready, grads, (f"{name}.bn.bias", f"{name}.bn.weight", f"{name}.input_conv.bias", f"{name}.input_conv.weight"))
    return dx


def generator_forward(P, x, mask, training=True, checkpoint=False, out=None):
    B, H, W = x.shape
    m, er, dmasks, dr = O.mask_pyramid(mask, [(k, s, p) for (_n, _ci, _co, k, s, p) in G_ENC],
                                       [(k, s, p) for (_n, _ci, _co, k, s, p) in G_DEC])

    enc_ctx, e = [], [x.reshape(B, H, W, 1)]
    for i, (name, _ci, _co, k, s, p) in enumerate(G_ENC):
        a, c = _pconv_fwd(P, name, k, s, p, e[-1], m[i], er[i + 1], training)
        e.append(a)
        enc_ctx.append(c)
    d, dec_ctx = e[7], []
    fshape = (B, H, W, G_DEC[6][2])
    bnin_final = BNIN_FINAL and O.conv_bnin_supported(fshape, 1, 3, 1, 1) and O.conv_bnin_supported(fshape, 1, 3, 1, 1, wgrad=True)
    up_c = None
    for i, (name, _ci, _co, k, s, p) in enumerate(G_DEC):
        skip = e[6 - i] if i < 6 else None
        Hs, Ws = (skip.shape[1], skip.shape[2]) if skip is not None else (H, W)
        if up_c is not None:
            up_shape = tuple(up_c.y.shape)
            cat = O.upcat_fwd(up_c.y, skip, Hs, Ws, out_mask=dmasks[i], up_bn=_bn_in(P, up_c))
        else:
            up_shape = tuple(d.shape)
            cat = O.upcat_fwd(d, skip, Hs, Ws, out_mask=dmasks[i])
        if i == 6:
            defer = bnin_final
        else:
            nskip = e[5 - i] if i < 5 else None
            nH, nW = (nskip.shape[1], nskip.shape[2]) if nskip is not None else (H, W)
            defer = BNIN_UPCAT and Hs * Ws * B > O.BN_SMALL_ROWS and \
                O.upcat_bn_supported((B, Hs, Ws, _co), None if nskip is None else tuple(nskip.shape), nH, nW)
        d, c = _pconv_fwd(P, name, k, s, p, cat, dmasks[i], dr[i], training, premasked=True, defer_act=defer)
        up_c = c if (defer and i < 6) else None
        c.up_shape, c.x_shape, c.skip_hw = up_shape, tuple(cat.shape), (Hs, Ws)
        if checkpoint:
            c.x = None
        dec_ctx.append(c)
    O.tag("final.fwd")
    if bnin_final:
        logits = O.conv_fwd_bnin(dec_ctx[6].y, _bn_in(P, dec_ctx[6]), P["final.weight"], P["final.bias"].detach(), 3, 1, 1)
    else:
        logits = O.conv_fwd(d, P["final.weight"], P["final.bias"].detach(), 3, 1, 1)
    out = O.sigmoid_composite_fwd(logits.reshape(B, H, W), x, mask, out=out)
    if PROBE is not None:
        PROBE("fwd", "final", logits)
        PROBE("fwd", "gen", out)
    if checkpoint:
        for i in range(1, 7):
            enc_ctx[i].x_shape = tuple(enc_ctx[i].x.shape)
            enc_ctx[i].x = None
        d = None
    return out, NS(enc=enc_ctx, dec=dec_ctx, d0=d, logits=logits, mask=mask, shape=(B, H, W), checkpoint=checkpoint,
                   bnin_final=bnin_final)


def _act_of(P, c):
    return O.bn_act_fwd(c.y, c.mean, c.rstd, P[f"{c.name}.bn.weight"], P[f"{c.name}.bn.bias"], O.ACT_RELU)


def _bn_in(P, c):
    return (c.mean, c.rstd, P[f"{c.name}.bn.weight"], P[f"{c.name}.bn.bias"], O.ACT_RELU, 0.0)


BNIN_FINAL = os.environ.get("TG_NO_BNIN") is None
BN_CONV1 = os.environ.get("TG_NO_BN_CONV1") is None
BNIN_UPCAT = os.environ.get("TG_NO_BNIN") is None and os.environ.get("TG_NO_BNIN_UPCAT") is None


def generator_backward(P, ctx, dout, want_dx=False, gbuf=None, on_ready=None):
    B, H, W = ctx.shape
    grads = {}
    ckpt = getattr(ctx, "checkpoint", False)
    dz, dx_comp = O.sigmoid_composite_bwd(dout, ctx.logits.reshape(B, H, W), ctx.mask, want_dx)
    dz = dz.reshape(B, H, W, 1)
    if PROBE is not None:
        PROBE("bwd", "gen", dout)
        PROBE("bwd", "final", dz)
    bnin = getattr(ctx, "bnin_final", False)
    d0 = ctx.dec[6].y if bnin else (_act_of(P, ctx.dec[6]) if ckpt else ctx.d0)
    fuse1 = BN_CONV1 and PROBE is None and O.bn_bwd_conv1_supported(tuple(d0.shape))
    if fuse1:
        da = None
    else:
        O.tag("final.dgrad")
        da = O.conv_dgrad(dz, P["final.weight"], tuple(d0.shape), 3, 1, 1)
    O.tag("final.wgrad")
    grads["final.weight"], grads["final.bias"] = _wgrad(gbuf, (d0, dz), lambda: O.conv_wgrad(
        d0, dz, P["final.weight"], 3, 1, 1, dw_out=gbuf["final.weight"] if gbuf is not None else None,
        db_out=gbuf["final.bias"] if gbuf is not None else None, in_bn=_bn_in(P, ctx.dec[6]) if bnin else None))
    _notify(on_ready, grads, ("final.bias", "final.weight"))
    del d0
    dskips = {}
    for i in range(6, -1, -1):
        c = ctx.dec[i]
        if ckpt:
            below = ctx.dec[i - 1] if i > 0 else ctx.enc[6]
            skip = _act_of(P, ctx.enc[5 - i]) if i < 6 else None
            if BNIN_UPCAT and O.upcat_bn_supported(tuple(below.y.shape), None if skip is None else tuple(skip.shape), *c.skip_hw):
                c.x = O.upcat_fwd(below.y, skip, c.skip_hw[0], c.skip_hw[1], out_mask=c.in_mask, up_bn=_bn_in(P, below))
            else:
                up_src = _act_of(P, below)
                c.x = O.upcat_fwd(up_src, skip, c.skip_hw[0], c.skip_hw[1], out_mask=c.in_mask)
                del up_src
            del skip
        dcat = _pconv_bwd(P, c, da, grads, gbuf=gbuf, on_ready=on_ready, conv1=(dz, P["final.weight"]) if (i == 6 and fuse1) else None)
        if ckpt:
            c.x = None
        _b, h, w, Cu = c.up_shape
        da, dskip = O.upcat_bwd(dcat, h, w, Cu)
        if i < 6:
            dskips[6 - i] = dskip
    dx = None
    for i in range(6, -1, -1):
        c = ctx.enc[i]
        if ckpt and i > 0:
            c.x = _act_of(P, ctx.enc[i - 1])
        if i > 0:
            da = _pconv_bwd(P, c, da, grads, dx_out=dskips[i], gbuf=gbuf, on_ready=on_ready)
            if ckpt:
                c.x = None
        else:
            dx = _pconv_bwd(P, c, da, grads, want_dx=want_dx, gbuf=gbuf, on_ready=on_ready)
    if want_dx:
        dx = O.axpby_(dx_comp, 1.0, 1.0, dx.reshape(B, H, W))
    join_side()
    return grads, dx


def discriminator_forward(P, img, training=True, groups=1, update_running=True):
    h = img if img.dim() == 4 else img.reshape(*img.shape, 1)
    Bg = h.shape[0] // groups
    assert Bg * groups == h.shape[0]
    layers = []
    for (ci, bi, _cin, _cout, k, s, p, leaky) in D_LAYERS:
        w, b = P[f"model.{ci}.weight"], P[f"model.{ci}.bias"].detach()
        O.tag(f"d{ci}.fwd")
        if bi is None:
            act = O.ACT_LEAKY if leaky else O.ACT_NONE
            a = O.conv_fwd(h, w, b, k, s, p, act=act, slope=0.2)
            layers.append(NS(ci=ci, bi=None, k=k, s=s, p=p, x=h, a=a, act=act))
        else:
            y = O.conv_fwd(h, w, b, k, s, p)
            if groups > 1 and training and y.shape[-1] % 4 == 0:
                mean2, rstd2, a = O.bn_fwd_grouped(y, groups, P[f"model.{bi}.weight"], P[f"model.{bi}.bias"], O.ACT_LEAKY, 0.2)
                if update_running:
                    O.bn_running_update_multi(mean2, rstd2, y.numel() // y.shape[-1] // groups, list(range(groups)),
                                              P[f"model.{bi}.running_mean"], P[f"model.{bi}.running_var"],
                                              P[f"model.{bi}.num_batches_tracked"])
                means, rstds = [mean2[gi] for gi in range(groups)], [rstd2[gi] for gi in range(groups)]
                layers.append(NS(ci=ci, bi=bi, k=k, s=s, p=p, x=h, y=y, mean=means[0], rstd=rstds[0], means=means, rstds=rstds,
                                 mean2=mean2, rstd2=rstd2, a=a))
                h = a
                continue
            a = torch.empty_like(y)
            means, rstds = [], []
            for gi in range(groups):
                yg, ag = y[gi * Bg:(gi + 1) * Bg], a[gi * Bg:(gi + 1) * Bg]
                if training:
                    run = (P[f"model.{bi}.running_mean"], P[f"model.{bi}.running_var"], P[f"model.{bi}.num_batches_tracked"]) \
                        if update_running else (None, None, None)
                    mean, rstd = O.bn_stats(yg, *run)
                else:
# ... 177 lines not shown
```

### terra-gan_amd/tg_hip/lib.py

```python
import ctypes as C
import os

import torch

_HERE = os.path.dirname(os.path.abspath(__file__))
LIB_PATH = os.environ.get("TG_HIP_LIB") or os.path.join(os.path.dirname(_HERE), "lib", "libterragan_hip.so")


class TgConv(C.Structure):
    _fields_ = [(n, C.c_int32) for n in ("B", "H", "W", "Cin", "Ho", "Wo", "Cout", "k", "stride", "pad", "precision")]


TG_MASK_PYRAMID_MAX = 24


class TgMaskOp(C.Structure):
    _fields_ = [(n, C.c_int32) for n in ("kind", "H", "W", "Ho", "Wo", "k", "stride", "pad")] + \
               [(n, C.c_void_p) for n in ("in_", "in2", "out", "out2")]


class TgMaskPyramid(C.Structure):
    _fields_ = [("nops", C.c_int32), ("_pad", C.c_int32), ("op", TgMaskOp * TG_MASK_PYRAMID_MAX)]


class TgBnAct(C.Structure):
    _fields_ = [(n, C.c_void_p) for n in ("mean", "rstd", "gamma", "beta")] + [("act", C.c_int32), ("slope", C.c_float)]


class TgSparseMap(C.Structure):
    _fields_ = [(n, C.c_void_p) for n in ("bits", "list", "count", "pix")] + [(n, C.c_int32) for n in ("nb", "tiles_y", "tiles_x", "_pad")]


class TgRasterPlan(C.Structure):
    _fields_ = [(n, C.c_int32) for n in ("H", "W", "wh", "ww", "overlap", "ny", "nx")]


TG_EVAL_MAX_CLASSES = 8


class TgAreaClasses(C.Structure):
    _fields_ = [("n_edges", C.c_int32), ("_pad", C.c_int32), ("px", C.c_int64 * (TG_EVAL_MAX_CLASSES - 1))]


class TgError(RuntimeError):
    pass


P, I, I64, F, SZ, D = C.c_void_p, C.c_int, C.c_int64, C.c_float, C.c_size_t, C.c_double
CP = C.POINTER(TgConv)
RP = C.POINTER(TgRasterPlan)

SIGNATURES = {
    "tg_version": (I, []),
    "tg_last_error": (C.c_char_p, []),
    "tg_conv_fwd_ws_bytes": (SZ, [CP]),
    "tg_conv_fwd": (I, [CP, P, P, P, P, P, I, F, P, P, SZ, P]),
    "tg_conv_dgrad_ws_bytes": (SZ, [CP]),
    "tg_conv_dgrad": (I, [CP, P, P, P, P, I, P, SZ, P]),
    "tg_conv_dgrad_gated": (I, [CP, P, P, P, P, I, F, P, P, SZ, P]),
    "tg_set_cu_reserve": (I, [I]),
    "tg_set_work_stealing": (I, [I]),
    "tg_conv_wprep_bytes": (SZ, [CP, I]),
    "tg_conv_wprep": (I, [CP, I, P, P, P]),
    "tg_conv_wprep_item_bytes": (SZ, []),
    "tg_conv_wprep_item": (I, [CP, I, P, P, P]),
    "tg_conv_wprep_run": (I, [P, I, P]),
    "tg_conv_fwd_p": (I, [CP, P, P, P, P, P, P, I, F, P, P, SZ, P]),
    "tg_conv_fwd_pool": (I, [CP, P, P, P, P, P, P, I, F, P, P, P, SZ, P]),
    "tg_conv_pool_code_supported": (I, [CP]),
    "tg_conv_fwd_pool_code": (I, [CP, P, P, P, P, P, P, P, SZ, P]),
    "tg_maxpool2_bwd_code": (I, [P, P, I, I, I, I, P, P]),
    "tg_vgg_sparse_map_bytes": (SZ, [I, I, I, C.c_char_p]),
    "tg_vgg_sparse_map": (I, [P, P, I, I, I, C.c_char_p, P, SZ, P, C.POINTER(TgSparseMap), P]),
    "tg_conv_dgrad_sparse": (I, [CP, P, P, P, P, I, F, P, P, C.POINTER(TgSparseMap), P, SZ, P]),
    "tg_conv_dgrad_sparse_planned": (I, [CP, I, C.POINTER(TgSparseMap)]),
    "tg_maxpool2_bwd_code_sparse": (I, [P, P, I, I, I, I, P, C.POINTER(TgSparseMap), P]),
    "tg_conv_fwd_sparse": (I, [CP, P, P, P, P, I, F, P, P, P, C.POINTER(TgSparseMap), P, SZ, P]),
    "tg_conv_bnin_supported": (I, [CP, I]),
    "tg_conv_fwd_bnin": (I, [CP, P, C.POINTER(TgBnAct), P, P, I, F, P, P, SZ, P]),
    "tg_conv_wgrad_bnin": (I, [CP, P, C.POINTER(TgBnAct), P, P, P, P, SZ, P]),
    "tg_conv_dgrad_p": (I, [CP, P, P, P, P, P, I, F, P, I, P, SZ, P]),
    "tg_relu_gate_pack": (I, [P, I64, I, P, P]),
    "tg_conv_dgrad_gbits": (I, [CP, P, P, P, P, P, P, I, P, SZ, P]),
    "tg_conv_wgrad_ws_bytes": (SZ, [CP]),
    "tg_conv_wgrad": (I, [CP, P, P, P, P, P, P, SZ, P]),
    "tg_fold_cin": (I, [P, I, I, I, P, P]),
    "tg_mask_update": (I, [P, I, I, I, I, I, I, I, I, P, P, P]),
    "tg_mask_up_merge": (I, [P, P, I, I, I, I, I, P, P]),
    "tg_mask_pyramid": (I, [C.POINTER(TgMaskPyramid), I, P]),
    "tg_bn_ws_bytes": (SZ, [I64, I]),
    "tg_bn_stats": (I, [P, I64, I, F, F, P, P, P, P, P, P, SZ, P]),
    "tg_bn_eval_stats": (I, [P, P, I, F, P, P, P]),
    "tg_bn_act_fwd": (I, [P, I64, I, P, P, P, P, I, F, P, P]),
    "tg_bn_fwd": (I, [P, I64, I, F, F, P, P, I, F, P, P, P, P, P, P, P, SZ, P]),
    "tg_bn_act_bwd": (I, [P, P, I64, I, P, P, P, P, I, F, P, P, P, P, P, P, SZ, P]),
    "tg_bn_bwd_conv1_supported": (I, [I64, I]),
    "tg_bn_conv1_ws_bytes": (SZ, [I64, I]),
    "tg_bn_act_bwd_conv1": (I, [P, P, I, I, I, P, I, P, P, P, P, I, F, P, P, P, P, P, P, SZ, P]),
    "tg_act_bwd": (I, [P, P, I64, I, I, F, P, P, P]),
    "tg_upcat_fwd": (I, [P, P, P, I, I, I, I, I, I, I, P, P]),
    "tg_upcat_bn_supported": (I, [I, I, I, I, I, I, I]),
    "tg_upcat_fwd_bn": (I, [P, C.POINTER(TgBnAct), P, P, I, I, I, I, I, I, I, P, P]),
    "tg_upcat_bwd": (I, [P, I, I, I, I, I, I, I, P, P, P]),
    "tg_sigmoid_composite_fwd": (I, [P, P, P, I64, P, P]),
    "tg_sigmoid_composite_bwd": (I, [P, P, P, I64, P, P, P]),
    "tg_maxpool2_fwd": (I, [P, I, I, I, I, P, P]),
    "tg_maxpool2_bwd": (I, [P, P, I, I, I, I, I, P, P]),
    "tg_pixel_loss_ws_bytes": (SZ, [I, I, I]),
    "tg_pixel_losses": (I, [P, P, P, P, I, I, I, F, F, F, F, P, P, P, I, P, SZ, P]),
    "tg_reduce_ws_bytes": (SZ, [I64]),
    "tg_l1_mean": (I, [P, P, I64, F, P, P, P, P, SZ, P]),
    "tg_l1_mean_relu": (I, [P, P, I64, F, P, P, P, P, SZ, P]),
    "tg_bce_logits": (I, [P, I64, F, F, P, P, P, P, SZ, P]),
    "tg_adam": (I, [P, P, P, P, I64, D, D, D, D, I, F, P]),
    "tg_adam_multi": (I, [P, P, I, I, D, D, D, D, I, F, P]),
    "tg_adam_scalars": (I, [D, D, D, I, P]),
    "tg_write_floats": (I, [P, I, P, P]),
    "tg_adam_multi_s": (I, [P, P, I, I, D, D, D, P, F, P]),
    "tg_axpby": (I, [P, F, F, P, I64, P]),
    "tg_lincomb": (I, [P, F, P, F, P, I64, P]),
    "tg_mul": (I, [P, P, P, I64, P]),
    "tg_mul_keep": (I, [P, P, P, P, I64, P]),
    "tg_bn_running_update": (I, [P, P, I64, I, F, F, P, P, P, P]),
    "tg_bn_grouped_ws_bytes": (SZ, [I64, I, I]),
    "tg_bn_fwd_grouped": (I, [P, I64, I, I, F, P, P, I, F, P, P, P, P, SZ, P]),
    "tg_bn_act_bwd_grouped": (I, [P, P, I64, I, I, P, P, P, P, I, F, P, P, P, P, P, SZ, P]),
    "tg_bn_running_update_multi": (I, [P, P, I64, I, F, F, C.POINTER(C.c_int), I, P, P, P, P]),
    "tg_quality_metrics_ws_bytes": (SZ, [I64, I, I]),
    "tg_quality_metrics": (I, [P, P, P, I64, I, I, P, P, SZ, P]),
    "tg_u8_to_tiles": (I, [P, P, I64, P, P, P]),
    "tg_raster_window_stats": (I, [P, P, RP, I, F, P, P, P, P]),
    "tg_raster_gather": (I, [P, P, RP, I, F, P, P, P, I, P, P, P]),
    "tg_raster_blend": (I, [P, P, RP, I, F, P, P, P, P, I, P, P, P]),
    "tg_hole_masks": (I, [P, P, I, I, P, P]),
    "tg_raster_sample": (I, [P, I64, I64, P, I, I, P, I, P, P, P, P]),
    "tg_objmask_known": (I, [P, P, I, I, I, F, P, P, P]),
    "tg_objmask_morph": (I, [P, P, I, I, I, I, P, P, P]),
    "tg_objmask_pmf_step": (I, [P, P, P, I, I, I, F, P, P, P, P, P]),
    "tg_objmask_components": (I, [P, I, I, P, P, P]),
    "tg_objmask_filter": (I, [P, P, P, I, I, I, I, P, P, P, P]),
    "tg_eval_holes": (I, [P, P, I, F, P, P, P, P, I, I, I, I, I, P, P, P, P]),
    "tg_hole_table": (I, [P, P, I, I, P, P, I, P, P]),
    "tg_terrain_errors_ws_bytes": (SZ, [I, I]),
    "tg_terrain_errors": (I, [P, P, P, I, F, P, P, P, P, P, I, I, I, D, C.POINTER(TgAreaClasses), P, P, P, P, SZ, P]),
    "tg_terrain_errors_finish": (I, [I, I, P, SZ, P, P]),
    "tg_select_f32_ws_bytes": (SZ, [I64, I]),
    "tg_select_f32": (I, [P, I64, P, I, P, P, SZ, P]),
    "tg_vfill_ws_bytes": (SZ, [I, I]),
    "tg_vfill_levels": (I, [I, I]),
    "tg_vfill_setup": (I, [P, P, I, F, I, I, P, SZ, P, P]),
    "tg_vfill_cycle": (I, [I, I, P, SZ, P, P]),
    "tg_vfill_finish": (I, [P, I, I, P, SZ, P, P]),
    "tg_seam_delta": (I, [P, P, I, F, P, I, I, I, P, P, P]),
    "tg_seam_apply": (I, [P, P, I, F, P, P, I, I, P, P]),
    "tg_prof_enable": (I, [I]),
    "tg_prof_summary": (I, [I, C.POINTER(C.c_double), C.POINTER(C.c_int64), C.POINTER(C.c_double), C.POINTER(C.c_double)]),
    "tg_prof_dump": (I, [C.c_char_p]),
    "tg_prof_tag": (I, [C.c_char_p]),
    "tg_nchw_to_nhwc": (I, [P, I, I, I, I, P, P]),
    "tg_nhwc_to_nchw": (I, [P, I, I, I, I, P, P]),
}

_lib = None


def load():
    global _lib
    if _lib is None:
        if not os.path.exists(LIB_PATH):
            raise TgError(f"{LIB_PATH} is missing: build it with `python terra-gan_amd/build.py` "
                          "(or __graft_entry__.build()); this framework has no CPU / eager fallback")
        lib = C.CDLL(LIB_PATH)
        for name, (res, args) in SIGNATURES.items():
            fn = getattr(lib, name)
            fn.restype, fn.argtypes = res, args
        _lib = lib
    return _lib


def check(rc, what=""):
    if rc != 0:
        raise TgError(f"{what} failed (rc={rc}): {load().tg_last_error().decode()}")
```

### terra-gan_amd/tg_hip/ops.py

```python
import ctypes as C

import torch

from . import lib as L

ACT_NONE, ACT_RELU, ACT_LEAKY = 0, 1, 2
PREC_F32, PREC_BF16, PREC_F32_WINO4 = 0, 1, 2
_precision = PREC_F32


def set_precision(name):
    global _precision
    _precision = {"f32": PREC_F32, "fp32": PREC_F32, "bf16": PREC_BF16}[name]


def get_precision():
    return "bf16" if _precision == PREC_BF16 else "f32"
BN_EPS, BN_MOMENTUM = 1e-5, 0.1
PROF_TAGS = False


def tag(name):
    if PROF_TAGS:
        _lib().tg_prof_tag(name.encode())
# ... 36 lines not shown


def empty(*shape, like=None, device=None):
    return torch.empty(*shape, dtype=torch.float32, device=like.device if like is not None else device)


def weight_view(w):
    v = w.detach().permute(0, 2, 3, 1)
    if not v.is_contiguous():
        w.data = w.data.contiguous(memory_format=torch.channels_last)
        v = w.detach().permute(0, 2, 3, 1)
        if not v.is_contiguous():
            dense = v.contiguous()
            w.data = dense.permute(0, 3, 1, 2)
            v = w.detach().permute(0, 2, 3, 1)
    return v


def _prec(wino4):
    return PREC_F32_WINO4 if (wino4 and _precision == PREC_F32) else _precision


def conv_geom(x, cout, k, stride, pad, wino4=False):
    B, H, W, Cin = x.shape
    Ho, Wo = (H + 2 * pad - k) // stride + 1, (W + 2 * pad - k) // stride + 1
    return L.TgConv(B, H, W, Cin, Ho, Wo, cout, k, stride, pad, _prec(wino4))


WPREP_FWD, WPREP_DGRAD = 0, 1
WPREP_CACHE = True
WPREP_VERIFY = __import__("os").environ.get("TG_WPREP_VERIFY") == "1"
WPREP_BATCH = True
_wprep = {}
_wstamp = {}
_wprep_tables = {}
wprep_capture_log = None


def weights_updated(params):
    ptrs = set()
    for p in params:
        if p.dim() == 4:
            ptr = p.data_ptr()
            _wstamp[ptr] = _wstamp.get(ptr, 0) + 1
            ptrs.add(ptr)
    if WPREP_BATCH and WPREP_CACHE and ptrs:
        _prepare_batch(ptrs)


def _prepare_batch(ptrs):
    ents = []
    for key, e in _wprep.items():
        if key[0] in ptrs and e[3] and e[4] and e[0]() is not None:
            ents.append((key, e))
    if not ents:
        return
    raw = b"".join(e[3] for _, e in ents)
    tkey = (ents[0][1][2].device, raw)
    table = _wprep_tables.get(tkey)
    if table is None:
        import numpy as np
        table = torch.from_numpy(np.frombuffer(raw, dtype=np.uint8).copy()).to(ents[0][1][2].device)
        if len(_wprep_tables) > 16:
            _wprep_tables.clear()
        _wprep_tables[tkey] = table
    L.check(_lib().tg_conv_wprep_run(C.c_void_p(table.data_ptr()), len(ents), _stream()), "tg_conv_wprep_run")
    for key, e in ents:
        e[1] = (e[0]()._version, _wstamp.get(key[0], 0))
        e[4] = False
    if wprep_capture_log is not None:
        wprep_capture_log.extend(key for key, _e in ents)


def graph_replayed(weight_ptrs, refreshed_keys):
    for ptr in weight_ptrs:
        _wstamp[ptr] = _wstamp.get(ptr, 0) + 1
    for key in refreshed_keys:
        e = _wprep.get(key)
        if e is not None:
            w = e[0]()
            if w is not None:
                e[1] = (w._version, _wstamp.get(key[0], 0))


def _prepared(w, wv, g, mode):
    if not WPREP_CACHE:
        return None
    import weakref
    ptr = wv.data_ptr()
    key = (ptr, mode, g.H, g.W, g.Cin, g.Cout, g.k, g.stride, g.pad, g.precision)
    stamp = (w._version, _wstamp.get(ptr, 0))
    ent = _wprep.get(key)
    if ent is not None and ent[0]() is w and ent[1] == stamp:
        ent[4] = True
        if WPREP_VERIFY and ent[2] is not None:
            fresh = torch.empty_like(ent[2])
            L.check(_lib().tg_conv_wprep(C.byref(g), mode, _p(wv), _p(fresh), _stream()), "tg_conv_wprep")
            if not torch.equal(fresh.view(torch.int32), ent[2].view(torch.int32)):
                raise L.TgError("prepared weights are stale: a parameter was rewritten without tg_hip.ops.weights_updated()")
        return ent[2]
    lib = _lib()
    if ent is None or ent[0]() is not w:
        nb = lib.tg_conv_wprep_bytes(C.byref(g), mode)
        buf = torch.empty((nb + 3) // 4, dtype=torch.float32, device=wv.device) if nb else None
        if len(_wprep) > 512:
            for k_ in [k_ for k_, e in _wprep.items() if e[0]() is None]:
                del _wprep[k_]
        item = False
        if buf is not None:
            raw = C.create_string_buffer(lib.tg_conv_wprep_item_bytes())
            if lib.tg_conv_wprep_item(C.byref(g), mode, _p(wv), _p(buf), raw):
                item = raw.raw
        ent = [weakref.ref(w), None, buf, item, True]
        _wprep[key] = ent
    if ent[2] is not None:
        L.check(lib.tg_conv_wprep(C.byref(g), mode, _p(wv), _p(ent[2]), _stream()), "tg_conv_wprep")
    ent[1] = stamp
    ent[4] = True
    return ent[2]


_sparse_tickets = {}


class SparseMaps:

    def __init__(self, buf, maps, for_bwd=False):
        self.buf, self.maps, self.for_bwd = buf, maps, for_bwd


def vgg_sparse_map(x, nb, plan, mask=None):
    _chk(x, "x"); _chk(mask, "mask")
    H, W = x.shape[1], x.shape[2]
    assert x.shape[0] == 2 * nb and x.numel() == 2 * nb * H * W, (tuple(x.shape), nb)
    assert mask is None or (mask.numel() == nb * H * W and mask.shape[0] == nb), (tuple(mask.shape), nb, H, W)
    lib = _lib()
    pb = plan.encode()
    nbytes = lib.tg_vgg_sparse_map_bytes(nb, H, W, pb)
    if nbytes == 0:
        return None
    dev = x.device.index if x.device.index is not None else torch.cuda.current_device()
    ticket = _sparse_tickets.get(dev)
    if ticket is None or ticket.numel() < nb + 1:
        if torch.cuda.is_current_stream_capturing():
            return None
        ticket = _sparse_tickets[dev] = torch.zeros(max(nb + 1, 64), dtype=torch.int32, device=x.device)
    buf = torch.empty(nbytes, dtype=torch.uint8, device=x.device)
    nconv = plan.count("C")
    maps = (L.TgSparseMap * nconv)()
    L.check(lib.tg_vgg_sparse_map(_p(x), _p(mask), nb, H, W, pb, _p(buf), nbytes, _p(ticket), maps, _stream()), "tg_vgg_sparse_map")
    return SparseMaps(buf, maps, for_bwd=mask is not None)


def conv_fwd(x, w, bias, k, stride, pad, in_mask=None, ratio=None, act=ACT_NONE, slope=0.0, wino4=False, pool=False, sparse=None):
    _chk(x, "x"); _chk(bias, "bias"); _chk(in_mask, "in_mask"); _chk(ratio, "ratio")
    if sparse is not None:
        assert in_mask is None and ratio is None
        wv = weight_view(w)
        _chk(wv, "weight")
        g = conv_geom(x, wv.shape[0], k, stride, pad, wino4)
        y = empty(g.B, g.Ho, g.Wo, g.Cout, like=x)
        yp = empty(g.B, g.Ho // 2, g.Wo // 2, g.Cout, like=x) if pool else None
        lib = _lib()
        ws = workspace(lib.tg_conv_fwd_ws_bytes(C.byref(g)))
        L.check(lib.tg_conv_fwd_sparse(C.byref(g), _p(x), _p(wv), _p(_prepared(w, wv, g, WPREP_FWD)), _p(bias), act, slope, _p(y),
                                       _p(yp), None, C.byref(sparse), _p(ws), ws.numel() * 4, _stream()), "tg_conv_fwd_sparse")
        return (y, yp) if pool else y
    wv = weight_view(w)
    _chk(wv, "weight")
    g = conv_geom(x, wv.shape[0], k, stride, pad, wino4)
    assert wv.shape == (g.Cout, k, k, g.Cin), (tuple(wv.shape), g.Cout, k, g.Cin)
    y = empty(g.B, g.Ho, g.Wo, g.Cout, like=x)
    lib = _lib()
    nb = lib.tg_conv_fwd_ws_bytes(C.byref(g))
    ws = workspace(nb)
    if pool:
        yp = empty(g.B, g.Ho // 2, g.Wo // 2, g.Cout, like=x)
        L.check(lib.tg_conv_fwd_pool(C.byref(g), _p(x), _p(in_mask), _p(wv), _p(_prepared(w, wv, g, WPREP_FWD)), _p(bias), _p(ratio),
                                     act, slope, _p(y), _p(yp), _p(ws), ws.numel() * 4, _stream()), "tg_conv_fwd_pool")
        return y, yp
    L.check(lib.tg_conv_fwd_p(C.byref(g), _p(x), _p(in_mask), _p(wv), _p(_prepared(w, wv, g, WPREP_FWD)), _p(bias), _p(ratio),
                              act, slope, _p(y), _p(ws), ws.numel() * 4, _stream()), "tg_conv_fwd")
    return y


def _bn_act(in_bn):
    mean, rstd, gamma, beta = in_bn[:4]
    for t in (mean, rstd, gamma, beta):
        _chk(t, "in_bn")
    act = in_bn[4] if len(in_bn) > 4 else ACT_RELU
    slope = in_bn[5] if len(in_bn) > 5 else 0.0
    return L.TgBnAct(mean.data_ptr(), rstd.data_ptr(), gamma.detach().data_ptr(), beta.detach().data_ptr(), act, slope)


def conv_bnin_supported(x_shape, cout, k, stride, pad, wgrad=False):
    B, H, W, Cin = x_shape
    Ho, Wo = (H + 2 * pad - k) // stride + 1, (W + 2 * pad - k) // stride + 1
    g = L.TgConv(B, H, W, Cin, Ho, Wo, cout, k, stride, pad, _precision)
    return bool(_lib().tg_conv_bnin_supported(C.byref(g), 1 if wgrad else 0))


def conv_fwd_bnin(x, in_bn, w, bias, k, stride, pad, act=ACT_NONE, slope=0.0):
    _chk(x, "x"); _chk(bias, "bias")
    wv = weight_view(w)
    _chk(wv, "weight")
    g = conv_geom(x, wv.shape[0], k, stride, pad)
    y = empty(g.B, g.Ho, g.Wo, g.Cout, like=x)
    lib = _lib()
    ws = workspace(lib.tg_conv_fwd_ws_bytes(C.byref(g)))
    bn = _bn_act(in_bn)
    L.check(lib.tg_conv_fwd_bnin(C.byref(g), _p(x), C.byref(bn), _p(wv), _p(bias), act, slope, _p(y), _p(ws), ws.numel() * 4, _stream()),
            "tg_conv_fwd_bnin")
    return y


def conv_pool_code_supported(x_shape, cout):
    B, H, W, Cin = x_shape
    g = L.TgConv(B, H, W, Cin, H, W, cout, 3, 1, 1, _precision)
    return bool(_lib().tg_conv_pool_code_supported(C.byref(g)))


def conv_fwd_pool_code(x, w, bias, sparse=None):
    _chk(x, "x"); _chk(bias, "bias")
    wv = weight_view(w)
    _chk(wv, "weight")
    g = conv_geom(x, wv.shape[0], 3, 1, 1)
    yp = empty(g.B, g.Ho // 2, g.Wo // 2, g.Cout, like=x)
    code = torch.empty((g.B, g.Ho // 2, g.Wo // 2, g.Cout), dtype=torch.uint8, device=x.device)
    lib = _lib()
    ws = workspace(lib.tg_conv_fwd_ws_bytes(C.byref(g)))
    if sparse is not None:
        L.check(lib.tg_conv_fwd_sparse(C.byref(g), _p(x), _p(wv), _p(_prepared(w, wv, g, WPREP_FWD)), _p(bias), ACT_RELU, 0.0, None,
                                       _p(yp), C.c_void_p(code.data_ptr()), C.byref(sparse), _p(ws), ws.numel() * 4, _stream()),
                "tg_conv_fwd_sparse")
        return yp, code
    L.check(lib.tg_conv_fwd_pool_code(C.byref(g), _p(x), _p(wv), _p(_prepared(w, wv, g, WPREP_FWD)), _p(bias), _p(yp),
                                      C.c_void_p(code.data_ptr()), _p(ws), ws.numel() * 4, _stream()), "tg_conv_fwd_pool_code")
    return yp, code


def maxpool2_bwd_code(dout, code, sparse=None, out=None):
    _chk(dout, "dout"); _chk(out, "out")
    B, Ho, Wo, Cc = dout.shape
    assert code.dtype == torch.uint8 and code.is_contiguous() and tuple(code.shape[1:]) == (Ho, Wo, Cc) and code.shape[0] >= B
    dx = out if out is not None else empty(B, 2 * Ho, 2 * Wo, Cc, like=dout)
    assert tuple(dx.shape) == (B, 2 * Ho, 2 * Wo, Cc)
    if sparse is not None:
        L.check(_lib().tg_maxpool2_bwd_code_sparse(_p(dout), C.c_void_p(code.data_ptr()), B, Ho, Wo, Cc, _p(dx), C.byref(sparse), _stream()),
                "tg_maxpool2_bwd_code_sparse")
        return dx
    L.check(_lib().tg_maxpool2_bwd_code(_p(dout), C.c_void_p(code.data_ptr()), B, Ho, Wo, Cc, _p(dx), _stream()), "tg_maxpool2_bwd_code")
    return dx


def conv_dgrad_sparse_planned(x_shape, cout, sparse, gate=0):
    B, H, W, Cin = x_shape
    g = L.TgConv(B, H, W, Cin, H, W, cout, 3, 1, 1, _precision)
    return bool(_lib().tg_conv_dgrad_sparse_planned(C.byref(g), gate, C.byref(sparse)))


def relu_gate_pack(a, nb=None):
    _chk(a, "a")
    B, H, W, Cc = a.shape
    nb = B if nb is None else nb
    assert 0 < nb <= B, (nb, B)
    bits = torch.empty((nb, H, W, Cc // 32), dtype=torch.uint32, device=a.device)
    L.check(_lib().tg_relu_gate_pack(_p(a), nb * H * W, Cc, C.c_void_p(bits.data_ptr()), _stream()), "tg_relu_gate_pack")
    return bits


def conv_dgrad(dy, w, x_shape, k, stride, pad, in_mask=None, out=None, gate=None, gate_act=ACT_RELU, gate_slope=0.0, wino4=False,
               gate_bits=None, sparse=None):
    _chk(dy, "dy"); _chk(in_mask, "in_mask"); _chk(out, "out"); _chk(gate, "gate")
    wv = weight_view(w)
    B, H, W, Cin = x_shape
    g = L.TgConv(B, H, W, Cin, dy.shape[1], dy.shape[2], dy.shape[3], k, stride, pad, _prec(wino4))
    acc = 1 if out is not None else 0
    dx = out if out is not None else empty(B, H, W, Cin, like=dy)
    lib = _lib()
    ws = workspace(lib.tg_conv_dgrad_ws_bytes(C.byref(g)))
    if sparse is not None:
        assert in_mask is None and not wino4 and tuple(dx.shape) == tuple(x_shape)
        assert gate is None or (gate_bits is None and tuple(gate.shape) == tuple(x_shape))
        if gate_bits is not None:
            assert gate_bits.dtype == torch.uint32 and gate_bits.is_contiguous() and tuple(gate_bits.shape) == (B, H, W, Cin // 32), \
                (gate_bits.dtype, tuple(gate_bits.shape), tuple(x_shape))
        L.check(lib.tg_conv_dgrad_sparse(C.byref(g), _p(dy), _p(wv), _p(_prepared(w, wv, g, WPREP_DGRAD)), _p(gate),
                                         gate_act if gate is not None else ACT_NONE, gate_slope,
                                         C.c_void_p(gate_bits.data_ptr()) if gate_bits is not None else None, _p(dx),
                                         C.byref(sparse), _p(ws), ws.numel() * 4, _stream()), "tg_conv_dgrad_sparse")
        return dx
    if gate_bits is not None:
        assert gate is None and out is None, "conv_dgrad: gate_bits is exclusive with gate and does not accumulate"
        assert gate_bits.dtype == torch.uint32 and gate_bits.is_contiguous() and tuple(gate_bits.shape) == (B, H, W, Cin // 32), \
            (gate_bits.dtype, tuple(gate_bits.shape), tuple(x_shape))
        L.check(lib.tg_conv_dgrad_gbits(C.byref(g), _p(dy), _p(wv), _p(_prepared(w, wv, g, WPREP_DGRAD)), _p(in_mask),
                                        C.c_void_p(gate_bits.data_ptr()), _p(dx), 0, _p(ws), ws.numel() * 4, _stream()),
                "tg_conv_dgrad_gbits")
        return dx
    if gate is not None:
        assert out is None and tuple(gate.shape) == tuple(x_shape)
    L.check(lib.tg_conv_dgrad_p(C.byref(g), _p(dy), _p(wv), _p(_prepared(w, wv, g, WPREP_DGRAD)), _p(in_mask), _p(gate),
                                gate_act if gate is not None else ACT_NONE, gate_slope, _p(dx), acc, _p(ws), ws.numel() * 4,
                                _stream()), "tg_conv_dgrad")
    return dx


def conv_wgrad(x, dy, w, k, stride, pad, in_mask=None, want_bias=True, dw_out=None, db_out=None, in_bn=None):
    _chk(x, "x"); _chk(dy, "dy"); _chk(in_mask, "in_mask")
    wv = weight_view(w)
    B, H, W, Cin = x.shape
    g = L.TgConv(B, H, W, Cin, dy.shape[1], dy.shape[2], dy.shape[3], k, stride, pad, _precision)
    if dw_out is not None:
        dwv = dw_out.permute(0, 2, 3, 1)
        assert dwv.is_contiguous() and dwv.shape == wv.shape
    else:
        dwv = torch.empty_like(wv)
    db = (db_out if db_out is not None else empty(g.Cout, like=x)) if want_bias else None
    lib = _lib()
    ws = workspace(lib.tg_conv_wgrad_ws_bytes(C.byref(g)))
    if in_bn is not None:
        assert in_mask is None
        bn = _bn_act(in_bn)
        L.check(lib.tg_conv_wgrad_bnin(C.byref(g), _p(x), C.byref(bn), _p(dy), _p(dwv), _p(db), _p(ws), ws.numel() * 4, _stream()),
                "tg_conv_wgrad_bnin")
        return dwv.permute(0, 3, 1, 2), db
    L.check(lib.tg_conv_wgrad(C.byref(g), _p(x), _p(in_mask), _p(dy), _p(dwv), _p(db), _p(ws), ws.numel() * 4, _stream()),
            "tg_conv_wgrad")
    return dwv.permute(0, 3, 1, 2), db


def fold_cin(w):
    wv = weight_view(w)
    co, kh, kw, ci = wv.shape
    out = empty(co, kh, kw, 1, like=wv)
    L.check(_lib().tg_fold_cin(_p(wv), co, kh * kw, ci, _p(out), _stream()), "tg_fold_cin")
    return out.permute(0, 3, 1, 2)


def mask_update(mask, k, stride, pad):
    _chk(mask, "mask")
    B, H, W = mask.shape
    Ho, Wo = (H + 2 * pad - k) // stride + 1, (W + 2 * pad - k) // stride + 1
    mo, ratio = empty(B, Ho, Wo, like=mask), empty(B, Ho, Wo, like=mask)
    L.check(_lib().tg_mask_update(_p(mask), B, H, W, k, stride, pad, Ho, Wo, _p(mo), _p(ratio), _stream()), "tg_mask_update")
    return mo, ratio


def mask_up_merge(up_mask, skip_mask):
    _chk(up_mask, "up_mask"); _chk(skip_mask, "skip_mask")
    B, h, w = up_mask.shape
    _, H, W = skip_mask.shape
    out = torch.empty_like(skip_mask)
    L.check(_lib().tg_mask_up_merge(_p(up_mask), _p(skip_mask), B, h, w, H, W, _p(out), _stream()), "tg_mask_up_merge")
    return out


MASK_FUSE_PIXELS = 64 * 64


def mask_pyramid(mask, enc, dec):
    _chk(mask, "mask")
    B, H, W = mask.shape
    ne, nd = len(enc), len(dec)
    dims = [(H, W)]
    for (k, s, p) in enc:
        h, w = dims[-1]
        dims.append(((h + 2 * p - k) // s + 1, (w + 2 * p - k) // s + 1))
    sizes = [B * h * w for (h, w) in dims[1:]] * 2
    ddims = []
    cur = dims[ne]
    for j, (k, s, p) in enumerate(dec):
        sk = dims[ne - 1 - j]
        ddims.append((cur, sk))
        cur = ((sk[0] + 2 * p - k) // s + 1, (sk[1] + 2 * p - k) // s + 1)
        sizes += [B * sk[0] * sk[1], B * cur[0] * cur[1], B * cur[0] * cur[1]]
    offs, tot = [], 0
    for n in sizes:
        offs.append(tot)
        tot += (n + 63) // 64 * 64
    buf = torch.empty(tot, dtype=torch.float32, device=mask.device)
    it = iter(zip(offs, sizes))

    def view(shape):
        o, n = next(it)
        return buf[o:o + n].view(shape)

    m, er = [mask], [None]
    mo_views = [view((B,) + dims[i + 1]) for i in range(ne)]
    r_views = [view((B,) + dims[i + 1]) for i in range(ne)]
    pm = L.TgMaskPyramid()
    n_ops = 0
    lib = _lib()

    def flush():
        nonlocal n_ops, pm
        if n_ops:
            pm.nops = n_ops
            L.check(lib.tg_mask_pyramid(C.byref(pm), B, _stream()), "tg_mask_pyramid")
            pm, n_ops = L.TgMaskPyramid(), 0

    def put(kind, hin, hout, k, s, p, a, a2, o, o2):
        nonlocal n_ops
        if hout[0] * hout[1] > MASK_FUSE_PIXELS:
            flush()
            if kind == 0:
                L.check(lib.tg_mask_update(_p(a), B, hin[0], hin[1], k, s, p, hout[0], hout[1], _p(o), _p(o2), _stream()), "tg_mask_update")
            else:
                L.check(lib.tg_mask_up_merge(_p(a), _p(a2), B, hin[0], hin[1], hout[0], hout[1], _p(o), _stream()), "tg_mask_up_merge")
            return
        if n_ops == L.TG_MASK_PYRAMID_MAX:
            flush()
        op = pm.op[n_ops]
        op.kind, op.H, op.W, op.Ho, op.Wo, op.k, op.stride, op.pad = kind, hin[0], hin[1], hout[0], hout[1], k, s, p
        op.in_, op.in2, op.out, op.out2 = a.data_ptr(), (a2.data_ptr() if a2 is not None else None), o.data_ptr(), \
            (o2.data_ptr() if o2 is not None else None)
        n_ops += 1

    for i, (k, s, p) in enumerate(enc):
        put(0, dims[i], dims[i + 1], k, s, p, m[-1], None, mo_views[i], r_views[i])
        m.append(mo_views[i])
        er.append(r_views[i])
    dm, dmasks, dr = m[ne], [], []
    for j, (k, s, p) in enumerate(dec):
        (hin, sk) = ddims[j]
        skip_m = m[ne - 1 - j]
        mm = view((B,) + sk)
        hout = ((sk[0] + 2 * p - k) // s + 1, (sk[1] + 2 * p - k) // s + 1)
        mo, r = view((B,) + hout), view((B,) + hout)
        put(1, hin, sk, 0, 0, 0, dm, skip_m, mm, None)
        put(0, sk, hout, k, s, p, mm, None, mo, r)
        dmasks.append(mm)
        dr.append(r)
        dm = mo
    flush()
    return m, er, dmasks, dr


BN_SMALL_ROWS = 2048


def bn_stats(y, running_mean=None, running_var=None, nbt=None, eps=BN_EPS, momentum=BN_MOMENTUM):
    _chk(y, "y")
    Cc = y.shape[-1]
    rows = y.numel() // Cc
    mean, rstd = empty(Cc, like=y), empty(Cc, like=y)
    lib = _lib()
    ws = workspace(lib.tg_bn_ws_bytes(rows, Cc))
    nbt_p = None if nbt is None else C.c_void_p(nbt.data_ptr())
    L.check(lib.tg_bn_stats(_p(y), rows, Cc, eps, momentum, _p(mean), _p(rstd), _p(running_mean), _p(running_var), nbt_p,
                            _p(ws), ws.numel() * 4, _stream()), "tg_bn_stats")
    return mean, rstd


def bn_fwd(y, gamma, beta, act, slope=0.0, running_mean=None, running_var=None, nbt=None, out=None, eps=BN_EPS,
           momentum=BN_MOMENTUM, apply=True):
    _chk(y, "y"); _chk(out, "out")
    Cc = y.shape[-1]
    rows = y.numel() // Cc
    mean, rstd = empty(Cc, like=y), empty(Cc, like=y)
    if out is None and apply:
        out = torch.empty_like(y)
    lib = _lib()
    ws = workspace(lib.tg_bn_ws_bytes(rows, Cc))
    nbt_p = None if nbt is None else C.c_void_p(nbt.data_ptr())
    L.check(lib.tg_bn_fwd(_p(y), rows, Cc, eps, momentum, _p(gamma.detach()), _p(beta.detach()), act, slope, _p(mean), _p(rstd),
                          _p(running_mean), _p(running_var), nbt_p, _p(out), _p(ws), ws.numel() * 4, _stream()), "tg_bn_fwd")
    return mean, rstd, out


def bn_eval_stats(running_mean, running_var, eps=BN_EPS):
    Cc = running_mean.numel()
    mean, rstd = torch.empty_like(running_mean), torch.empty_like(running_mean)
    L.check(_lib().tg_bn_eval_stats(_p(running_mean), _p(running_var), Cc, eps, _p(mean), _p(rstd), _stream()), "tg_bn_eval_stats")
    return mean, rstd


def bn_running_update(mean, rstd, rows, running_mean, running_var, nbt, eps=BN_EPS, momentum=BN_MOMENTUM):
# ... 712 lines not shown
```

Baseline: 1075 tiles/s.

## Keep space-to-depth input from forward for wgrad and fuse wide Winograd reduce

```diff
diff --git a/include/terragan_hip.h b/include/terragan_hip.h
--- a/include/terragan_hip.h
+++ b/include/terragan_hip.h
@@ -92,10 +92,16 @@
 
 int tg_set_cu_reserve(int cus);
 int tg_set_work_stealing(int mode);
+int tg_set_wgrad_reduce(int mode);
 
 size_t tg_conv_wgrad_ws_bytes(const TgConv* g);
 int tg_conv_wgrad(const TgConv* g, const float* x, const float* in_mask, const float* dy,
                   float* dw, float* db, float* ws, size_t ws_bytes, tg_stream_t stream);
+size_t tg_conv_s2d_bytes(const TgConv* g);
+int tg_conv_fwd_s2d(const TgConv* g, const float* x, const float* in_mask, const float* w, const float* wprep, const float* bias,
+                    const float* ratio, int act, float slope, float* y, float* x2, float* ws, size_t ws_bytes, tg_stream_t stream);
+int tg_conv_wgrad_s2d(const TgConv* g, const float* x2, const float* dy, float* dw, float* db, float* ws, size_t ws_bytes,
+                      tg_stream_t stream);
 
 int tg_fold_cin(const float* w3, int cout, int taps, int cin, float* w1, tg_stream_t stream);
 
diff --git a/terra-gan_amd/csrc/igemm.hip b/terra-gan_amd/csrc/igemm.hip
--- a/terra-gan_amd/csrc/igemm.hip
+++ b/terra-gan_amd/csrc/igemm.hip
@@ -133,6 +133,12 @@
 extern "C" int tg_set_work_stealing(int mode) {
     TG_REQUIRE(mode >= 0 && mode <= 2, "tg_set_work_stealing: mode %d not in {0, 1, 2}", mode);
     g_work_stealing.store(mode, std::memory_order_relaxed);
+    return TG_OK;
+}
+static std::atomic<int> g_wgrad_reduce_wide{1};
+extern "C" int tg_set_wgrad_reduce(int mode) {
+    TG_REQUIRE(mode >= 0 && mode <= 2, "tg_set_wgrad_reduce: mode %d not in {0, 1, 2}", mode);
+    g_wgrad_reduce_wide.store(mode, std::memory_order_relaxed);
     return TG_OK;
 }
 constexpr int WQ_HOST_Z = 16, WQ_HOST_INTS = 8 * WQ_HOST_Z + 8, WQ_POOL_BLOCKS = 64;
@@ -1363,6 +1369,7 @@
     unsigned char* pool_code = nullptr;
     const BnIn* in_bn = nullptr;
     const TgSparseMap* sparse = nullptr;
+    float* x2_keep = nullptr;
     int pool_fused = 0;
 };
 static int conv_fwd_impl(const TgConv* g, const float* x, const float* in_mask, const float* w, float* wprep, int prep,
@@ -1393,7 +1400,7 @@
     if (s2d_ok(g) && (prep < 0 || ws_ok)) {
         hipStream_t s = (hipStream_t)stream;
         const TgConv g2 = s2d_geom(g);
-        float* x2 = ws;
+        float* x2 = ex && ex->x2_keep ? ex->x2_keep : ws;
         float* w2 = prep ? wprep : ws + s2d_x_floats(g);
         float* ws2 = ws ? ws + s2d_x_floats(g) + s2d_w_floats(g) : nullptr;
         if (prep < 0 && g_wprep_capture) {
@@ -1543,6 +1550,22 @@
                              tg_stream_t stream) {
     return conv_fwd_impl(g, x, in_mask, w, const_cast<float*>(wprep), wprep ? 1 : 0, bias, ratio, act, slope, y, ws, ws_bytes,
                          stream);
+}
+static bool s2d_wgrad_route(const TgConv* g);
+extern "C" size_t tg_conv_s2d_bytes(const TgConv* g) {
+    if (!g || check_conv(g, "tg_conv_s2d_bytes") || !s2d_ok(g) || !s2d_wgrad_route(g)) return 0;
+    return s2d_x_floats(g) * sizeof(float);
+}
+extern "C" int tg_conv_fwd_s2d(const TgConv* g, const float* x, const float* in_mask, const float* w, const float* wprep,
+                               const float* bias, const float* ratio, int act, float slope, float* y, float* x2, float* ws,
+                               size_t ws_bytes, tg_stream_t stream) {
+    TG_REQUIRE(g && x2 && aligned16(x2) && tg_conv_s2d_bytes(g) > 0, "tg_conv_fwd_s2d: not a space-to-depth layer (ask tg_conv_s2d_bytes first)");
+    TG_REQUIRE(ws && aligned16(ws) && ws_bytes >= tg_conv_fwd_ws_bytes(g), "tg_conv_fwd_s2d: workspace too small (%zu < %zu)", ws_bytes,
+               tg_conv_fwd_ws_bytes(g));
+    FwdExtras e;
+    e.x2_keep = x2;
+    return conv_fwd_impl(g, x, in_mask, w, const_cast<float*>(wprep), wprep ? 1 : 0, bias, ratio, act, slope, y, ws, ws_bytes,
+                         stream, nullptr, &e);
 }
 
 __global__ __launch_bounds__(256) void transpose_w_kernel(const float* __restrict__ w, float* __restrict__ wt,
@@ -2350,7 +2373,17 @@
 }
 
 static int conv_wgrad_impl(const TgConv* g, const float* x, const float* in_mask, const float* dy, float* dw, float* db, float* ws,
-                           size_t ws_bytes, tg_stream_t stream, const BnIn* in_bn);
+                           size_t ws_bytes, tg_stream_t stream, const BnIn* in_bn, const float* x2_kept = nullptr);
+static bool s2d_wgrad_route(const TgConv* g) {
+    if (!s2d_ok(g) || smallconv_wgrad_applies(wgrad_params(g))) return false;
+    const TgConv g2 = s2d_geom(g);
+    return wino16_wgrad_ok(&g2, nullptr) || wino_wgrad_ok(&g2, nullptr);
+}
+extern "C" int tg_conv_wgrad_s2d(const TgConv* g, const float* x2, const float* dy, float* dw, float* db, float* ws, size_t ws_bytes,
+                                 tg_stream_t stream) {
+    TG_REQUIRE(g && x2 && tg_conv_s2d_bytes(g) > 0, "tg_conv_wgrad_s2d: not a space-to-depth layer (ask tg_conv_s2d_bytes first)");
+    return conv_wgrad_impl(g, x2, nullptr, dy, dw, db, ws, ws_bytes, stream, nullptr, x2);
+}
 extern "C" int tg_conv_wgrad(const TgConv* g, const float* x, const float* in_mask, const float* dy, float* dw,
                              float* db, float* ws, size_t ws_bytes, tg_stream_t stream) {
     return conv_wgrad_impl(g, x, in_mask, dy, dw, db, ws, ws_bytes, stream, nullptr);
@@ -2363,7 +2396,7 @@
     return conv_wgrad_impl(g, x, nullptr, dy, dw, db, ws, ws_bytes, stream, &b);
 }
 static int conv_wgrad_impl(const TgConv* g, const float* x, const float* in_mask, const float* dy, float* dw, float* db, float* ws,
-                           size_t ws_bytes, tg_stream_t stream, const BnIn* in_bn) {
+                           size_t ws_bytes, tg_stream_t stream, const BnIn* in_bn, const float* x2_kept) {
     int rc = check_conv(g, "tg_conv_wgrad");
     if (rc) return rc;
     TG_REQUIRE(x && dy && dw && ws, "tg_conv_wgrad: null pointer");
@@ -2403,23 +2436,28 @@
         const TgConv g2 = s2d_geom(g);
         const bool w16 = wino16_wgrad_ok(&g2, nullptr);
         if (w16 || wino_wgrad_ok(&g2, nullptr)) {
-            float* x2 = ws;
+            const float* x2 = x2_kept ? x2_kept : ws;
             float* dw2 = ws + s2d_x_floats(g);
             float* wsr = dw2 + s2d_w_floats(g);
-            hipLaunchKernelGGL(s2d_kernel, dim3(ew_grid((int64_t)g->B * g->H * g->W * (g->Cin / 4), 256)), dim3(256), 0, s, x, in_mask,
-                               x2, g->B, g->H, g->W, g->Cin);
-            TG_CHECK_LAUNCH("s2d_kernel");
+            if (!x2_kept) {
+                hipLaunchKernelGGL(s2d_kernel, dim3(ew_grid((int64_t)g->B * g->H * g->W * (g->Cin / 4), 256)), dim3(256), 0, s, x, in_mask,
+                                   ws, g->B, g->H, g->W, g->Cin);
+                TG_CHECK_LAUNCH("s2d_kernel");
+            }
             WgradParams p2 = p;
             p2.x = x2; p2.amask = nullptr; p2.H = g2.H; p2.W = g2.W; p2.C = g2.Cin; p2.k = 3; p2.stride = 1; p2.pad = 1;
             p2.Ktot = 9 * g2.Cin;
+            int wrote5 = 0;
             {
                 AlgScale sc(25.0 / 36.0);
-                rc = w16 ? launch_wino16_wgrad(&g2, p2, dw2, wsr, s) : launch_wino_wgrad(&g2, p2, dw2, wsr, s);
+                rc = w16 ? launch_wino16_wgrad(&g2, p2, dw2, wsr, s, dw, &wrote5) : launch_wino_wgrad(&g2, p2, dw2, wsr, s, dw, &wrote5);
             }
             if (rc) return rc;
-            hipLaunchKernelGGL(w5x5_s2d_kernel, dim3(ew_grid((int64_t)g->Cout * 25 * g->Cin, 256)), dim3(256), 0, s, dw2, dw, g->Cout,
-                               g->Cin, 0);
-            TG_CHECK_LAUNCH("w5x5_s2d_kernel");
+            if (!wrote5) {
+                hipLaunchKernelGGL(w5x5_s2d_kernel, dim3(ew_grid((int64_t)g->Cout * 25 * g->Cin, 256)), dim3(256), 0, s, dw2, dw,
+                                   g->Cout, g->Cin, 0);
+                TG_CHECK_LAUNCH("w5x5_s2d_kernel");
+            }
             if (db) {
                 rc = colsum((size_t)(wsr - ws) + align_up(w16 ? wino16_wgrad_ws_floats(&g2) : wino_wgrad_ws_floats(&g2), 64));
                 if (rc) return rc;
diff --git a/terra-gan_amd/csrc/wino.inc b/terra-gan_amd/csrc/wino.inc
--- a/terra-gan_amd/csrc/wino.inc
+++ b/terra-gan_amd/csrc/wino.inc
@@ -1148,6 +1148,104 @@
     }
 }
 
+constexpr int WR_ELEMS = 32, WR_THREADS = 16 * WR_ELEMS;
+__device__ __attribute__((noinline)) void wino_wgrad_gtg(float* ue) {
+    float u[16];
+#pragma unroll
+    for (int i = 0; i < 16; ++i) u[i] = ue[i * WR_ELEMS];
+    float t[3][4];
+#pragma unroll
+    for (int b = 0; b < 4; ++b) {
+        t[0][b] = u[0 * 4 + b] + 0.5f * (u[1 * 4 + b] + u[2 * 4 + b]);
+        t[1][b] = 0.5f * (u[1 * 4 + b] - u[2 * 4 + b]);
+        t[2][b] = 0.5f * (u[1 * 4 + b] + u[2 * 4 + b]) + u[3 * 4 + b];
+    }
+#pragma unroll
+    for (int uu = 0; uu < 3; ++uu) {
+        ue[(uu * 3 + 0) * WR_ELEMS] = t[uu][0] + 0.5f * (t[uu][1] + t[uu][2]);
+        ue[(uu * 3 + 1) * WR_ELEMS] = 0.5f * (t[uu][1] - t[uu][2]);
+        ue[(uu * 3 + 2) * WR_ELEMS] = 0.5f * (t[uu][1] + t[uu][2]) + t[uu][3];
+    }
+}
+template <bool S2D5>
+__global__ __launch_bounds__(WR_THREADS) void wino_wgrad_reduce_wide_kernel(const float* __restrict__ slabs, float* __restrict__ dw,
+                                                                            int Cout, int Cin, int ntco, int ntci, int splits) {
+    __shared__ float us[16 * WR_ELEMS];
+    const int e = threadIdx.x & (WR_ELEMS - 1), pt = threadIdx.x / WR_ELEMS;
+    const int idx = blockIdx.x * WR_ELEMS + e;
+    const int col = idx & 63, row = (idx >> 6) & 63, tile = idx >> 12;
+    const size_t sstride = (size_t)ntci * ntco * 16 * 4096;
+    const float* sl = slabs + ((size_t)tile * 16 + pt) * 4096 + row * 64 + col;
+    float s = 0.f;
+    int sp = 0;
+    for (; sp + 16 <= splits; sp += 16) {
+        float v[16];
+#pragma unroll
+        for (int k = 0; k < 16; ++k) v[k] = sl[(size_t)(sp + k) * sstride];
+#pragma unroll
+        for (int k = 0; k < 16; ++k) s += v[k];
+    }
+    for (; sp + 4 <= splits; sp += 4) {
+        float v[4];
+#pragma unroll
+        for (int k = 0; k < 4; ++k) v[k] = sl[(size_t)(sp + k) * sstride];
+#pragma unroll
+        for (int k = 0; k < 4; ++k) s += v[k];
+    }
+    for (; sp < splits; ++sp) s += sl[(size_t)sp * sstride];
+    us[pt * WR_ELEMS + e] = s;
+    __syncthreads();
+    if (pt != 0) return;
+    wino_wgrad_gtg(us + e);
+    float out[9];
+#pragma unroll
+    for (int k = 0; k < 9; ++k) out[k] = us[k * WR_ELEMS + e];
+    const int tco = tile % ntco, tci = tile / ntco;
+    const int co = tco * 64 + 4 * (row & 15) + (row >> 4), ci = tci * 64 + 4 * (col & 15) + (col >> 4);
+    if constexpr (!S2D5) {
+        float* o = dw + ((size_t)co * 9) * Cin + ci;
+#pragma unroll
+        for (int k = 0; k < 9; ++k) o[(size_t)k * Cin] = out[k];
+    } else {
+        const int C = Cin >> 2, ph = ci / C, c = ci - ph * C;
+        const int dy = ph >> 1, dx = ph & 1;
+        const auto rsrc = __builtin_amdgcn_make_buffer_rsrc(dw, 0, (int)((size_t)Cout * 25 * C * 4), 0x00020000);
+        const uint32_t OOB = 0xFFFFFFF0u, base = (uint32_t)((co * 25) * C + c) * 4u, tap = (uint32_t)C * 4u;
+#pragma unroll
+        for (int uu = 0; uu < 3; ++uu) {
+            const int ky = 2 * uu + dy;
+            const bool ok = ky < 5;
+            const uint32_t r = base + (uint32_t)(ky * 5 + dx) * tap;
+            __builtin_amdgcn_raw_buffer_store_b32(__builtin_bit_cast(uint32_t, out[uu * 3 + 0]), rsrc, ok ? r : OOB, 0, 0);
+            __builtin_amdgcn_raw_buffer_store_b32(__builtin_bit_cast(uint32_t, out[uu * 3 + 1]), rsrc, ok ? r + 2 * tap : OOB, 0, 0);
+            __builtin_amdgcn_raw_buffer_store_b32(__builtin_bit_cast(uint32_t, out[uu * 3 + 2]), rsrc, ok && dx == 0 ? r + 4 * tap : OOB, 0, 0);
+        }
+    }
+}
+static int launch_wino_wgrad_reduce(const TgConv* g, const WinoWgradGeom& q, const float* ws, float* dw, float* dw5, int* wrote5,
+                                    hipStream_t s) {
+    if (wrote5) *wrote5 = 0;
+    const int mode = g_wgrad_reduce_wide.load(std::memory_order_relaxed);
+    const bool five = dw5 && (size_t)g->Cout * 25 * (g->Cin / 4) * 4 < ((size_t)1 << 31);
+    if (mode == 2 || (mode == 1 && (five || (int64_t)g->Cout * g->Cin / 256 < WINO_PLAN_CUS))) {
+        const int grid = (int)((int64_t)g->Cout * g->Cin / WR_ELEMS);
+        if (five) {
+            hipLaunchKernelGGL(wino_wgrad_reduce_wide_kernel<true>, dim3(grid), dim3(WR_THREADS), 0, s, ws, dw5, g->Cout, g->Cin,
+                               q.ntco, q.ntci, q.splits);
+            if (wrote5) *wrote5 = 1;
+        } else {
+            hipLaunchKernelGGL(wino_wgrad_reduce_wide_kernel<false>, dim3(grid), dim3(WR_THREADS), 0, s, ws, dw, g->Cout, g->Cin,
+                               q.ntco, q.ntci, q.splits);
+        }
+        TG_CHECK_LAUNCH("wino_wgrad_reduce_wide_kernel");
+        return TG_OK;
+    }
+    hipLaunchKernelGGL(wino_wgrad_reduce_kernel, dim3(ew_grid((int64_t)g->Cout * g->Cin, 256)), dim3(256), 0, s, ws, dw, g->Cout,
+                       g->Cin, q.ntco, q.ntci, q.splits);
+    TG_CHECK_LAUNCH("wino_wgrad_reduce_kernel");
+    return TG_OK;
+}
+
 static bool wino_wgrad_ok(const TgConv* g, const float* in_mask) {
     static const bool off = getenv("TG_NO_WINO") != nullptr || getenv("TG_NO_WINO_WGRAD") != nullptr;
     if (off || in_mask != nullptr) return false;
@@ -1177,7 +1275,8 @@
     const WinoWgradGeom q = wino_wgrad_plan(g);
     return (size_t)q.splits * q.ntco * q.ntci * 16 * 4096;
 }
-static int launch_wino_wgrad(const TgConv* g, const WgradParams& p, float* dw, float* ws, hipStream_t s) {
+static int launch_wino_wgrad(const TgConv* g, const WgradParams& p, float* dw, float* ws, hipStream_t s, float* dw5 = nullptr,
+                             int* wrote5 = nullptr) {
     const WinoWgradGeom q = wino_wgrad_plan(g);
     const size_t lds = (size_t)WINO_WG_LDS_FLOATS * sizeof(float);
     static LdsOptIn opt;
@@ -1188,8 +1287,5 @@
         hipLaunchKernelGGL(wino_wgrad_kernel, dim3(q.ntco * q.ntci * q.splits), dim3(WINO_THREADS), lds, s, p, q, ws);
     }
     TG_CHECK_LAUNCH("wino_wgrad_kernel");
-    hipLaunchKernelGGL(wino_wgrad_reduce_kernel, dim3(ew_grid((int64_t)g->Cout * g->Cin, 256)), dim3(256), 0, s, ws, dw, g->Cout,
-                       g->Cin, q.ntco, q.ntci, q.splits);
-    TG_CHECK_LAUNCH("wino_wgrad_reduce_kernel");
-    return TG_OK;
-}
+    return launch_wino_wgrad_reduce(g, q, ws, dw, dw5, wrote5, s);
+}
diff --git a/terra-gan_amd/csrc/wino16.inc b/terra-gan_amd/csrc/wino16.inc
--- a/terra-gan_amd/csrc/wino16.inc
+++ b/terra-gan_amd/csrc/wino16.inc
@@ -774,7 +774,8 @@
     const WinoWgradGeom q = wino16_wgrad_plan(g);
     return (size_t)q.splits * q.ntco * q.ntci * 16 * 4096;
 }
-static int launch_wino16_wgrad(const TgConv* g, const WgradParams& p, float* dw, float* ws, hipStream_t s) {
+static int launch_wino16_wgrad(const TgConv* g, const WgradParams& p, float* dw, float* ws, hipStream_t s, float* dw5 = nullptr,
+                               int* wrote5 = nullptr) {
     const WinoWgradGeom q = wino16_wgrad_plan(g);
     static LdsOptIn opt;
     if (int rc = lds_opt_in(opt, reinterpret_cast<const void*>(wino16_wgrad_kernel), W16G_LDS_BYTES, "wino16 wgrad")) return rc;
@@ -784,8 +785,5 @@
         hipLaunchKernelGGL(wino16_wgrad_kernel, dim3(q.ntco * q.ntci * q.splits), dim3(WINO_THREADS), W16G_LDS_BYTES, s, p, q, ws);
     }
     TG_CHECK_LAUNCH("wino16_wgrad_kernel");
-    hipLaunchKernelGGL(wino_wgrad_reduce_kernel, dim3(ew_grid((int64_t)g->Cout * g->Cin, 256)), dim3(256), 0, s, ws, dw, g->Cout,
-                       g->Cin, q.ntco, q.ntci, q.splits);
-    TG_CHECK_LAUNCH("wino_wgrad_reduce_kernel");
-    return TG_OK;
-}
+    return launch_wino_wgrad_reduce(g, q, ws, dw, dw5, wrote5, s);
+}
diff --git a/terra-gan_amd/tg_hip/engine.py b/terra-gan_amd/tg_hip/engine.py
--- a/terra-gan_amd/tg_hip/engine.py
+++ b/terra-gan_amd/tg_hip/engine.py
@@ -21,6 +21,7 @@
 VGG_WINO4_MINCH = int(os.environ.get("TG_VGG_WINO4_MINCH", "128"))
 VGG_SPARSE = os.environ.get("TG_VGG_SPARSE", "1") != "0"
 VGG_SPARSE_BWD = os.environ.get("TG_VGG_SPARSE_BWD", "1") != "0"
+KEEP_S2D = True
 POOL_CODE = os.environ.get("TG_NO_POOL_CODE") is None
 
 
@@ -63,10 +64,12 @@
         torch.cuda.current_stream().wait_stream(_side_stream())
 
 
-def _pconv_fwd(P, name, k, s, p, x, in_mask, ratio, training, premasked=False, defer_act=False):
+def _pconv_fwd(P, name, k, s, p, x, in_mask, ratio, training, premasked=False, defer_act=False, keep_s2d=False):
     O.tag(f"{name}.fwd")
-    y = O.conv_fwd(x, P[f"{name}.input_conv.weight"], P[f"{name}.input_conv.bias"].detach(), k, s, p,
-                   in_mask=None if premasked else in_mask, ratio=ratio)
+    y, x2 = O.conv_fwd(x, P[f"{name}.input_conv.weight"], P[f"{name}.input_conv.bias"].detach(), k, s, p,
+                       in_mask=None if premasked else in_mask, ratio=ratio, keep_s2d=True) if keep_s2d and k == 5 else \
+        (O.conv_fwd(x, P[f"{name}.input_conv.weight"], P[f"{name}.input_conv.bias"].detach(), k, s, p,
+                    in_mask=None if premasked else in_mask, ratio=ratio), None)
     if training:
         mean, rstd, a = O.bn_fwd(y, P[f"{name}.bn.weight"], P[f"{name}.bn.bias"], O.ACT_RELU, 0.0, P[f"{name}.bn.running_mean"],
                                  P[f"{name}.bn.running_var"], P[f"{name}.bn.num_batches_tracked"], apply=not defer_act)
@@ -76,7 +79,7 @@
     if PROBE is not None:
         PROBE("fwd", name, a if a is not None else O.bn_act_fwd(y, mean, rstd, P[f"{name}.bn.weight"], P[f"{name}.bn.bias"], O.ACT_RELU))
     return a, NS(name=name, k=k, s=s, p=p, x=x, in_mask=in_mask, ratio=ratio, y=y, mean=mean, rstd=rstd,
-                 premasked=premasked)
+                 premasked=premasked, x2=x2)
 
 
 def _notify(on_ready, grads, keys):
@@ -103,7 +106,7 @@
     O.tag(f"{name}.wgrad")
     dw, _ = _wgrad(gbuf, (c.x, dyr, wmask), lambda: O.conv_wgrad(
         c.x, dyr, P[f"{name}.input_conv.weight"], c.k, c.s, c.p, in_mask=wmask, want_bias=False,
-        dw_out=gbuf[f"{name}.input_conv.weight"] if gbuf is not None else None))
+        dw_out=gbuf[f"{name}.input_conv.weight"] if gbuf is not None else None, x_s2d=getattr(c, "x2", None)))
     grads[f"{name}.input_conv.weight"], grads[f"{name}.input_conv.bias"] = dw, db
     grads[f"{name}.bn.weight"], grads[f"{name}.bn.bias"] = dgamma, dbeta
     _notify(on_ready, grads, (f"{name}.bn.bias", f"{name}.bn.weight", f"{name}.input_conv.bias", f"{name}.input_conv.weight"))
@@ -117,7 +120,7 @@
 
     enc_ctx, e = [], [x.reshape(B, H, W, 1)]
     for i, (name, _ci, _co, k, s, p) in enumerate(G_ENC):
-        a, c = _pconv_fwd(P, name, k, s, p, e[-1], m[i], er[i + 1], training)
+        a, c = _pconv_fwd(P, name, k, s, p, e[-1], m[i], er[i + 1], training, keep_s2d=KEEP_S2D and training and not checkpoint)
         e.append(a)
         enc_ctx.append(c)
     d, dec_ctx = e[7], []
diff --git a/terra-gan_amd/tg_hip/lib.py b/terra-gan_amd/tg_hip/lib.py
--- a/terra-gan_amd/tg_hip/lib.py
+++ b/terra-gan_amd/tg_hip/lib.py
@@ -60,6 +60,7 @@
     "tg_conv_dgrad_gated": (I, [CP, P, P, P, P, I, F, P, P, SZ, P]),
     "tg_set_cu_reserve": (I, [I]),
     "tg_set_work_stealing": (I, [I]),
+    "tg_set_wgrad_reduce": (I, [I]),
     "tg_conv_wprep_bytes": (SZ, [CP, I]),
     "tg_conv_wprep": (I, [CP, I, P, P, P]),
     "tg_conv_wprep_item_bytes": (SZ, []),
@@ -84,6 +85,9 @@
     "tg_conv_dgrad_gbits": (I, [CP, P, P, P, P, P, P, I, P, SZ, P]),
     "tg_conv_wgrad_ws_bytes": (SZ, [CP]),
     "tg_conv_wgrad": (I, [CP, P, P, P, P, P, P, SZ, P]),
+    "tg_conv_s2d_bytes": (SZ, [CP]),
+    "tg_conv_fwd_s2d": (I, [CP, P, P, P, P, P, P, I, F, P, P, P, SZ, P]),
+    "tg_conv_wgrad_s2d": (I, [CP, P, P, P, P, P, SZ, P]),
     "tg_fold_cin": (I, [P, I, I, I, P, P]),
     "tg_mask_update": (I, [P, I, I, I, I, I, I, I, I, P, P, P]),
     "tg_mask_up_merge": (I, [P, P, I, I, I, I, I, P, P]),
diff --git a/terra-gan_amd/tg_hip/ops.py b/terra-gan_amd/tg_hip/ops.py
--- a/terra-gan_amd/tg_hip/ops.py
+++ b/terra-gan_amd/tg_hip/ops.py
@@ -212,7 +212,8 @@
     return SparseMaps(buf, maps, for_bwd=mask is not None)
 
 
-def conv_fwd(x, w, bias, k, stride, pad, in_mask=None, ratio=None, act=ACT_NONE, slope=0.0, wino4=False, pool=False, sparse=None):
+def conv_fwd(x, w, bias, k, stride, pad, in_mask=None, ratio=None, act=ACT_NONE, slope=0.0, wino4=False, pool=False, sparse=None,
+             keep_s2d=False):
     _chk(x, "x"); _chk(bias, "bias"); _chk(in_mask, "in_mask"); _chk(ratio, "ratio")
     if sparse is not None:
         assert in_mask is None and ratio is None
@@ -239,9 +240,16 @@
         L.check(lib.tg_conv_fwd_pool(C.byref(g), _p(x), _p(in_mask), _p(wv), _p(_prepared(w, wv, g, WPREP_FWD)), _p(bias), _p(ratio),
                                      act, slope, _p(y), _p(yp), _p(ws), ws.numel() * 4, _stream()), "tg_conv_fwd_pool")
         return y, yp
+    if keep_s2d:
+        nx2 = lib.tg_conv_s2d_bytes(C.byref(g))
+        if nx2:
+            x2 = torch.empty(nx2 // 4, dtype=torch.float32, device=x.device)
+            L.check(lib.tg_conv_fwd_s2d(C.byref(g), _p(x), _p(in_mask), _p(wv), _p(_prepared(w, wv, g, WPREP_FWD)), _p(bias), _p(ratio),
+                                        act, slope, _p(y), _p(x2), _p(ws), ws.numel() * 4, _stream()), "tg_conv_fwd_s2d")
+            return y, x2
     L.check(lib.tg_conv_fwd_p(C.byref(g), _p(x), _p(in_mask), _p(wv), _p(_prepared(w, wv, g, WPREP_FWD)), _p(bias), _p(ratio),
                               act, slope, _p(y), _p(ws), ws.numel() * 4, _stream()), "tg_conv_fwd")
-    return y
+    return (y, None) if keep_s2d else y
 
 
 def _bn_act(in_bn):
@@ -366,7 +374,7 @@
     return dx
 
 
-def conv_wgrad(x, dy, w, k, stride, pad, in_mask=None, want_bias=True, dw_out=None, db_out=None, in_bn=None):
+def conv_wgrad(x, dy, w, k, stride, pad, in_mask=None, want_bias=True, dw_out=None, db_out=None, in_bn=None, x_s2d=None):
     _chk(x, "x"); _chk(dy, "dy"); _chk(in_mask, "in_mask")
     wv = weight_view(w)
     B, H, W, Cin = x.shape
@@ -384,6 +392,12 @@
         bn = _bn_act(in_bn)
         L.check(lib.tg_conv_wgrad_bnin(C.byref(g), _p(x), C.byref(bn), _p(dy), _p(dwv), _p(db), _p(ws), ws.numel() * 4, _stream()),
                 "tg_conv_wgrad_bnin")
+        return dwv.permute(0, 3, 1, 2), db
+    if x_s2d is not None:
+        assert x_s2d.is_contiguous() and x_s2d.dtype == torch.float32 and x_s2d.numel() * 4 == lib.tg_conv_s2d_bytes(C.byref(g)), \
+            (x_s2d.numel(), tuple(x.shape))
+        L.check(lib.tg_conv_wgrad_s2d(C.byref(g), _p(x_s2d), _p(dy), _p(dwv), _p(db), _p(ws), ws.numel() * 4, _stream()),
+                "tg_conv_wgrad_s2d")
         return dwv.permute(0, 3, 1, 2), db
     L.check(lib.tg_conv_wgrad(C.byref(g), _p(x), _p(in_mask), _p(dy), _p(dwv), _p(db), _p(ws), ws.numel() * 4, _stream()),
             "tg_conv_wgrad")
```

Result: no change. 1083 tiles/s, median of 6 (+0.7%).
